# cfpark00/vdm4cdm

Measured on NVIDIA B200. Metric: denoiser voxel-steps/s at 128^3 (reverse ancestral sampling), higher is better.
Workload: dtype bf16

## Files before the change

__graft_entry__.py:

```python
from __future__ import annotations

import os
import subprocess
import sys

ROOT = os.path.dirname(os.path.abspath(__file__))
if ROOT not in sys.path:
    sys.path.insert(0, ROOT)


def build() -> None:
    subprocess.run(["make", "-C", os.path.join(ROOT, "vdm4cdm_b200", "csrc"), "-j", "8"], check=True)
    os.makedirs(os.path.join(ROOT, "tools", "bin"), exist_ok=True)
    subprocess.run(["nvcc", "-gencode", "arch=compute_100a,code=sm_100a", "-O3", "-std=c++17", "-lineinfo", "-o",
                    os.path.join(ROOT, "tools", "bin", "probe_umma"), os.path.join(ROOT, "tools", "probe_umma.cu")],
                   check=True)
    import vdm4cdm_b200
    from vdm4cdm_b200 import _C
    lib = _C.lib()
    missing = [n for n in _C.declared_symbols() if not hasattr(lib, n)]
    if missing:
        raise RuntimeError(f"libvdm4cdm_b200.so does not export {missing}")
    import oracle


def smoke() -> None:
    import numpy as np
    import torch

    from oracle import power_ref
    from oracle.unet_ref import CUNet as RefNet
    from oracle.vdm_ref import VDM as RefVDM
    from vdm4cdm_b200 import _C, utils
    from vdm4cdm_b200.networks import CUNet
    from vdm4cdm_b200.vdm_model import VDM

    _C.check(_C.lib().vdm_device_supported(0), "vdm_device_supported")
    torch.manual_seed(0)
    shape, chs, b = (1, 16, 16, 16), (16, 32), 2
    kw = dict(shape=shape, chs=chs, s_conditioning_channels=1, v_conditioning_dims=[6], t_conditioning=True)
    ref = RefNet(**kw).eval()
    net = CUNet(**kw)
    net.load_state_dict(ref.state_dict())
    net = net.cuda().eval()
    g = torch.Generator().manual_seed(1)
    x = torch.randn((b,) + shape, generator=g)
    cond = 0.7 * x + 0.3 * torch.randn((b,) + shape, generator=g)
    t = torch.rand(b, generator=g)
    v = [torch.rand(b, 6, generator=g)]
    with torch.no_grad():
        want = ref(x, t=t, s_conditioning=cond, v_conditionings=v)
        got = net(x.cuda(), t=t.cuda(), s_conditioning=cond.cuda(), v_conditionings=[v[0].cuda()]).cpu()
    err = ((got - want).norm() / want.norm()).item()
    assert err < 1e-2, f"denoiser output differs from the oracle: relative L2 {err}"

    noises = [torch.randn((b,) + shape, generator=g) for _ in range(4)]
    vdm, ref_vdm = VDM(net).cuda().eval(), RefVDM(ref).eval()
    xs = vdm.sample(b, 3, "cuda:0", noise_fn=lambda d, s: noises[d].cuda(), s_conditioning=cond.cuda(),
                    v_conditionings=[v[0].cuda()]).cpu()
    with torch.no_grad():
        xr = ref_vdm.sample(b, 3, "cpu", noise_fn=lambda d, s: noises[d], s_conditioning=cond, v_conditionings=v)
    err_s = ((xs - xr).norm() / xr.norm()).item()
    assert err_s < 5e-2, f"3-step sample differs from the oracle: relative L2 {err_s}"

    from oracle.vdm_ref import LightVDM as RefLight
    from vdm4cdm_b200.vdm_model import LightVDM
    ref_l, mod_l = RefLight(ref).train(), LightVDM(net).cuda().train()
    for m in (ref, net):
        for blk in m.modules():
            if isinstance(blk, torch.nn.Dropout):
                blk.p = 0.0
    net.dropout_prob = 0.0
    for _, blk in net._blocks():
        blk.dropout_prob = 0.0
    times = torch.tensor([0.3, 0.8])
    loss_r, _ = ref_l.get_loss({"x": x, "conditioning": cond, "conditioning_values": v}, noise=noises[0], noise0=noises[1], times=times)
    loss_r.backward()
    loss_c, _ = mod_l.get_loss({"x": x.cuda(), "conditioning": cond.cuda(), "conditioning_values": [v[0].cuda()]},
                               noise=noises[0].cuda(), noise0=noises[1].cuda(), times=times.cuda())
    loss_c.backward()
    num = den = 0.0
    refp = dict(ref_l.named_parameters())
    for n_, p_ in mod_l.named_parameters():
        if p_.grad is not None and refp[n_].grad is not None:
            num += (p_.grad.cpu() - refp[n_].grad).double().pow(2).sum().item()
            den += refp[n_].grad.double().pow(2).sum().item()
    err_g = (num / den) ** 0.5
    assert abs(loss_c.item() - loss_r.item()) < 1e-2 * abs(loss_r.item()), (loss_c.item(), loss_r.item())
    assert err_g < 3e-2, f"training gradients differ from oracle autograd: relative L2 {err_g}"

    f1 = np.random.default_rng(2).standard_normal((2, 1, 32, 32, 32), dtype=np.float32)
    f2 = (0.7 * f1 + 0.3 * np.random.default_rng(3).standard_normal(f1.shape, dtype=np.float32)).astype(np.float32)
    k, p, n = utils.pk(torch.from_numpy(f1).cuda())
    ko, po, no = power_ref.pk(f1)
    assert np.array_equal(n.cpu().numpy(), no) and np.allclose(p.cpu().numpy(), po, rtol=1e-5)
    _, cc = utils.get_ccs(torch.from_numpy(f1).cuda(), torch.from_numpy(f2).cuda())
    assert np.allclose(cc.cpu().numpy(), power_ref.get_ccs(f1, f2)[1], atol=2e-5)
    torch.cuda.synchronize()
    print(f"smoke ok: denoiser rel-L2 {err:.2e}, 3-step sample rel-L2 {err_s:.2e}, VDM loss {loss_c.item():.4f} vs {loss_r.item():.4f}, "
          f"gradient rel-L2 {err_g:.2e}, P(k)/r(k) match")


if __name__ == "__main__":
    build()
    import torch
    if torch.cuda.is_available():
        smoke()
```

vdm4cdm_b200/csrc/conv3d.cu:

```cuda
#include "common.cuh"
#include "ptx.cuh"
#include "tma_host.cuh"

#ifdef VDM_BRINGUP
#define VDM_DBG(p, f) (((p).debug_flags & (f)) != 0)
#else
#define VDM_DBG(p, f) (false)
#endif

namespace vdm {

constexpr int kConvThreads = 512;
constexpr int kEpiThreads = 256;
constexpr int kEpiFirst = 128;
constexpr int kXfThreads = 128;
constexpr int kXfFirst = 384;
constexpr int kRegsWg0 = 64, kRegsEpi = 176, kRegsXf = 88;
constexpr int kXfGroup = 2;
constexpr int kResSlotBytes = 2 * 16 * kEpiThreads;
constexpr int kMaxBStages = 16;
constexpr int kMaxAStages = 4;
constexpr int kTileH = 16, kTileW = 8;

struct ConvKernelParams {
  int B, D, H, W;
  int c_out;
  int n_cta, n_split;
  int n_pad;
  int n_taps, pad;
  uint16_t tap16[VDM_MAX_TAPS];
  int8_t tap_kd[VDM_MAX_TAPS];
  int8_t tap_khw[VDM_MAX_TAPS];
  int8_t tap_of[3][9];
  int fold_streamed;
  int MT, KC, k_chunks;
  int Hd, Hh, Wh;
  int tiles_w, tiles_h, tiles_d, n_tiles;
  int fast_div_ok;
  float inv_n_split, inv_tiles_w, inv_tiles_h, inv_tiles_d;
  int a_stage_bytes, b_stage_bytes, nsb, taps_per_stage;
  int nsa;
  int b_resident;
  int plane_bytes;
  int tmem_cols;
  int x_planes, x_plane0, c_in8;
  int x_shift;
  int skip_chunks;
  int x2_planes, x2_plane0;
  int skip_w_bytes;
  const __nv_bfloat16* w2;
  const __nv_bfloat16* w;
  void* y;
  int y_planes, y_plane0, out_fp32;
  const float* chan_add;
  const int32_t* step_ptr;
  long long chan_add_step_stride;
  const __nv_bfloat16* residual;
  int r_planes, r_plane0;
  int r_up;
  int r_d2s_planes;
  int res_depth;
  int res_ring_off;
  double* stats;
  int stats_channels, stats_c0;
  const float* in_norm;
  int c_in;
  int xf_coef_off;
  int m_units, m_nseg, m_seglen;
  int debug_flags;
};

struct ConvShared {
  uint64_t a_full[kMaxAStages], a_empty[kMaxAStages];
  uint64_t a_ready[kMaxAStages];
  uint64_t b_full[kMaxBStages], b_empty[kMaxBStages];
  uint64_t tmem_full[2], tmem_empty[2];
  uint32_t tmem_base;
  alignas(16) float cadd[2][256];
};

__device__ __forceinline__ void warp_column_sums16(float (&v)[16]) {
  const unsigned full = 0xffffffffu;
  const int lane = threadIdx.x & 31;
#pragma unroll
  for (int i = 0; i < 8; ++i) {
    const bool hi = lane & 16;
    const float send = hi ? v[i] : v[i + 8];
    const float keep = hi ? v[i + 8] : v[i];
    v[i] = keep + __shfl_xor_sync(full, send, 16);
  }
#pragma unroll
  for (int i = 0; i < 4; ++i) {
    const bool hi = lane & 8;
    const float send = hi ? v[i] : v[i + 4];
    const float keep = hi ? v[i + 4] : v[i];
    v[i] = keep + __shfl_xor_sync(full, send, 8);
  }
#pragma unroll
  for (int i = 0; i < 2; ++i) {
    const bool hi = lane & 4;
    const float send = hi ? v[i] : v[i + 2];
    const float keep = hi ? v[i + 2] : v[i];
    v[i] = keep + __shfl_xor_sync(full, send, 4);
  }
  {
    const bool hi = lane & 2;
    const float send = hi ? v[0] : v[1];
    const float keep = hi ? v[1] : v[0];
    v[0] = keep + __shfl_xor_sync(full, send, 2);
  }
  v[0] += __shfl_xor_sync(full, v[0], 1);
}

struct TileCoord {
  int b, d0, h0, w0, ns;
};
__device__ __forceinline__ int fast_div(int x, int d, float inv) {
  (void)d;
  return __float2int_rz(((float)x + 0.5f) * inv);
}
__device__ __forceinline__ TileCoord decode_tile(const ConvKernelParams& p, int tile) {
  TileCoord t;
  int q;
  if (p.fast_div_ok) {
    q = fast_div(tile, p.n_split, p.inv_n_split); t.ns = tile - q * p.n_split; tile = q;
    q = fast_div(tile, p.tiles_w, p.inv_tiles_w); t.w0 = (tile - q * p.tiles_w) * kTileW; tile = q;
    q = fast_div(tile, p.tiles_h, p.inv_tiles_h); t.h0 = (tile - q * p.tiles_h) * kTileH; tile = q;
    q = fast_div(tile, p.tiles_d, p.inv_tiles_d); t.d0 = (tile - q * p.tiles_d) * p.MT;
    t.b = q;
  } else {
    t.ns = tile % p.n_split; tile /= p.n_split;
    t.w0 = (tile % p.tiles_w) * kTileW; tile /= p.tiles_w;
    t.h0 = (tile % p.tiles_h) * kTileH; tile /= p.tiles_h;
    t.d0 = (tile % p.tiles_d) * p.MT;
    t.b = tile / p.tiles_d;
  }
  return t;
}

struct Ring {
  uint32_t s, ph, n;
  __device__ __forceinline__ explicit Ring(uint32_t n_) : s(0u), ph(0u), n(n_) {}
  __device__ __forceinline__ void next() {
    if (++s == n) {
      s = 0u;
      ph ^= 1u;
    }
  }
};
__device__ __forceinline__ uint32_t hold_u32(uint32_t v) {
  asm volatile("mov.u32 %0, %0;" : "+r"(v));
  return v;
}

__device__ __forceinline__ uint64_t make_planar_desc(uint32_t smem_addr, uint32_t lbo, uint32_t sbo) {
  uint64_t d = 0;
  d |= (uint64_t)((smem_addr & 0x3FFFFu) >> 4);
  d |= (uint64_t)((lbo >> 4) & 0x3FFFu) << 16;
  d |= (uint64_t)((sbo >> 4) & 0x3FFFu) << 32;
  d |= (uint64_t)1 << 46;
  return d;
}

template <int MT, int KJ, int NF, bool FIRST>
__device__ __forceinline__ void issue_fold_tile(uint32_t a_lo0, uint32_t b_base16, uint64_t a_hi, uint64_t b_hi,
                                                uint32_t d_tmem0) {
  constexpr int Hh = kTileH + 2, Wh = kTileW + 2, Hd = MT + 2;
  constexpr uint32_t plane16 = (uint32_t)(Hd * Hh * Wh);
  constexpr uint32_t kstep_a16 = 2u * plane16;
  const uint32_t a_hi32 = (uint32_t)(a_hi >> 32), b_hi32 = (uint32_t)(b_hi >> 32);
#pragma unroll 1
  for (int i = 0; i < MT + 2; ++i) {
    const int kd_lo = (i - MT + 1) > 0 ? (i - MT + 1) : 0;
    const int kd_hi = i < 2 ? i : 2;
    const int s_lo = i - kd_hi;
    const int nblk = kd_hi - kd_lo + 1;
    const bool starts = FIRST && i < MT;
    const uint32_t a_i = a_lo0 + (uint32_t)(i * Hh * Wh) + (uint32_t)a_hi;
    const uint32_t b_i = b_base16 + (uint32_t)((2 - kd_hi) * NF) + (uint32_t)b_hi;
    const uint32_t d_i = d_tmem0 + (uint32_t)(s_lo * NF);
    const uint32_t idesc_i = ptx::make_idesc_bf16(128, (uint32_t)(nblk * NF));
#pragma unroll
    for (int khw = 0; khw < 9; ++khw) {
#pragma unroll
      for (int j = 0; j < KJ; ++j) {
        const uint32_t a_off = (uint32_t)((khw / 3) * Wh + khw % 3) + (uint32_t)j * kstep_a16;
        const uint32_t b_off = (uint32_t)((khw * 2 * KJ + 2 * j) * 3 * NF);
        if (khw == 0 && j == 0) {
          if (starts) {
            if (nblk > 1)
              ptx::umma_bf16_off(d_i, 0u, a_i, a_off, a_hi32, b_i, b_off, b_hi32,
                                 ptx::make_idesc_bf16(128, (uint32_t)((nblk - 1) * NF)), 1u);
            ptx::umma_bf16_off(d_tmem0, (uint32_t)(i * NF), a_i, a_off, a_hi32, b_i, b_off + (uint32_t)((nblk - 1) * NF), b_hi32,
                               ptx::make_idesc_bf16(128, (uint32_t)NF), 0u);
          } else {
            ptx::umma_bf16_off(d_i, 0u, a_i, a_off, a_hi32, b_i, b_off, b_hi32, idesc_i, 1u);
          }
        } else {
          ptx::umma_bf16_off(d_i, 0u, a_i, a_off, a_hi32, b_i, b_off, b_hi32, idesc_i, 1u);
        }
      }
    }
  }
}

template <int MT, int KJ, int NF>
__device__ __forceinline__ void issue_skip_chunk(uint32_t a_lo0, uint32_t b_lo16, uint32_t d_tmem0) {
  constexpr uint32_t slice16 = (uint32_t)(kTileH * kTileW);
  constexpr uint32_t plane16 = (uint32_t)MT * slice16;
  constexpr uint32_t kstep_a16 = 2u * plane16;
  const uint64_t a_hi = make_planar_desc(0, plane16 * 16u, (uint32_t)kTileW * 16u);
  const uint64_t b_hi = make_planar_desc(0, (uint32_t)NF * 16u, 128u);
  const uint32_t a_hi32 = (uint32_t)(a_hi >> 32), b_hi32 = (uint32_t)(b_hi >> 32);
  const uint32_t idesc = ptx::make_idesc_bf16(128, (uint32_t)NF);
  const uint32_t b_i = b_lo16 + (uint32_t)b_hi;
#pragma unroll
  for (int i = 0; i < MT; ++i) {
    const uint32_t a_i = a_lo0 + (uint32_t)i * slice16 + (uint32_t)a_hi;
#pragma unroll
    for (int j = 0; j < KJ; ++j)
      ptx::umma_bf16_off(d_tmem0, (uint32_t)(i * NF), a_i, (uint32_t)j * kstep_a16, a_hi32, b_i, (uint32_t)(2 * j * NF),
                         b_hi32, idesc, 1u);
  }
}

template <int MT, int KJ, int NF>
__device__ __forceinline__ void issue_fold_stage(uint32_t a_lo, uint32_t b_lo, uint32_t a_hi32, uint32_t b_hi32,
                                                 uint32_t d_tmem0, bool first) {
  constexpr int Hh = kTileH + 2, Wh = kTileW + 2, Hd = MT + 2;
  constexpr uint32_t plane16 = (uint32_t)(Hd * Hh * Wh);
  constexpr uint32_t kstep_a16 = 2u * plane16;
#pragma unroll
  for (int i = 0; i < MT + 2; ++i) {
    const int kd_lo = (i - MT + 1) > 0 ? (i - MT + 1) : 0;
    const int kd_hi = i < 2 ? i : 2;
    const int s_lo = i - kd_hi;
    const int nblk = kd_hi - kd_lo + 1;
#pragma unroll
    for (int j = 0; j < KJ; ++j) {
      const uint32_t a_off = (uint32_t)(i * Hh * Wh) + (uint32_t)j * kstep_a16;
      const uint32_t b_off = (uint32_t)((2 * j * 3 + (2 - kd_hi)) * NF);
      if (j == 0 && i < MT && first) {
        if (nblk > 1)
          ptx::umma_bf16_off(d_tmem0, (uint32_t)(s_lo * NF), a_lo, a_off, a_hi32, b_lo, b_off, b_hi32,
                             ptx::make_idesc_bf16(128, (uint32_t)((nblk - 1) * NF)), 1u);
        ptx::umma_bf16_off(d_tmem0, (uint32_t)(i * NF), a_lo, a_off, a_hi32, b_lo, b_off + (uint32_t)((nblk - 1) * NF), b_hi32,
                           ptx::make_idesc_bf16(128, (uint32_t)NF), 0u);
      } else {
        ptx::umma_bf16_off(d_tmem0, (uint32_t)(s_lo * NF), a_lo, a_off, a_hi32, b_lo, b_off, b_hi32,
                           ptx::make_idesc_bf16(128, (uint32_t)(nblk * NF)), 1u);
      }
    }
  }
}

template <int HH, int WH>
__device__ __forceinline__ bool halo_voxel_oob(int v, int dlo, int hlo, int wlo, int D, int H, int W) {
  const int dz = v / (HH * WH);
  const int rem = v - dz * (HH * WH);
  const int hy = rem / WH;
  const int wx = rem - hy * WH;
  return (unsigned)(dlo + dz) >= (unsigned)D || (unsigned)(hlo + hy) >= (unsigned)H || (unsigned)(wlo + wx) >= (unsigned)W;
}

__device__ __forceinline__ uint4 gn_silu8(const uint4 x, const float (&ca)[8], const float (&cb)[8]) {
  bf16x8 in;
  in.u = x;
  float f[8];
  unpack8(in, f);
#pragma unroll
  for (int j = 0; j < 8; ++j) {
    const float h = fmaf(f[j], ca[j], cb[j]);
    float t;
    asm("tanh.approx.f32 %0, %1;" : "=f"(t) : "f"(h));
    f[j] = fmaf(h, t, h);
  }
  return pack8(f).u;
}

template <int MT, int KJ>
__device__ __forceinline__ void transform_tiles(const ConvKernelParams& p, ConvShared* sh, uint8_t* a_smem, float* coef) {
  constexpr int planes = 2 * KJ;
  constexpr int nparts = planes >= 4 ? 1 : 4 / planes;
  static_assert((MT + 2) * (kTileH + 2) * (kTileW + 2) <= 64 * 32, "zmask: one bit per 16-byte unit of a thread");
  constexpr int pl_step = planes >= 4 ? 4 : planes;
  const int xt = threadIdx.x - kXfFirst, tw = xt >> 5, lane = xt & 31;
  const int pl0 = planes >= 4 ? tw : tw % planes;
  const int part = planes >= 4 ? 0 : tw / planes;
  const int vh = p.Hd * p.Hh * p.Wh;
  const int total_chunks = p.k_chunks + p.skip_chunks;
  int cur_b = -1;
  Ring ra((uint32_t)p.nsa);
  for (int tile = blockIdx.x; tile < p.n_tiles; tile += gridDim.x) {
    const TileCoord t = decode_tile(p, tile);
    if (t.b != cur_b) {
      asm volatile("bar.sync 3, 128;" ::: "memory");
      const float4* src = reinterpret_cast<const float4*>(p.in_norm + (long long)t.b * p.c_in * 2);
      for (int i = xt; i < p.c_in / 2; i += kXfThreads) reinterpret_cast<float4*>(coef)[i] = __ldg(src + i);
      asm volatile("bar.sync 3, 128;" ::: "memory");
      cur_b = t.b;
    }
    const int dlo = t.d0 - p.pad + p.x_shift, hlo = t.h0 - p.pad + p.x_shift, wlo = t.w0 - p.pad + p.x_shift;
    unsigned long long zmask = 0ull;
    if (dlo < 0 || dlo + p.Hd > p.D || hlo < 0 || hlo + p.Hh > p.H || wlo < 0 || wlo + p.Wh > p.W) {
      int k = 0;
      for (int idx = part * 32 + lane; idx < vh; idx += 32 * nparts, ++k) {
        const bool oob = p.pad ? halo_voxel_oob<kTileH + 2, kTileW + 2>(idx, dlo, hlo, wlo, p.D, p.H, p.W)
                               : halo_voxel_oob<kTileH, kTileW>(idx, dlo, hlo, wlo, p.D, p.H, p.W);
        if (oob) zmask |= 1ull << k;
      }
    }
    for (int kc = 0; kc < total_chunks; ++kc, ra.next()) {
      const int s = (int)ra.s;
      ptx::mbar_wait(&sh->a_full[s], ra.ph);
      if (kc < p.k_chunks && !VDM_DBG(p, 64)) {
        uint8_t* stage = a_smem + (size_t)s * p.a_stage_bytes;
#pragma unroll 1
        for (int pl = pl0; pl < planes; pl += pl_step) {
          float ca[8], cb[8];
          {
            const float4* cs = reinterpret_cast<const float4*>(coef + (size_t)((kc * planes + pl) * 8) * 2);
#pragma unroll
            for (int j4 = 0; j4 < 4; ++j4) {
              const float4 c4 = cs[j4];
              ca[2 * j4] = c4.x; cb[2 * j4] = c4.y; ca[2 * j4 + 1] = c4.z; cb[2 * j4 + 1] = c4.w;
            }
          }
          uint4* base = reinterpret_cast<uint4*>(stage + (size_t)pl * p.plane_bytes);
          constexpr int G = kXfGroup;
          const int step = 32 * nparts;
          int v = part * 32 + lane;
          uint4 cur[G], nxt[G];
#pragma unroll
          for (int g2 = 0; g2 < G; ++g2) {
            const int idx = v + g2 * step;
            cur[g2] = idx < vh ? base[idx] : make_uint4(0u, 0u, 0u, 0u);
          }
          int k = 0;
#pragma unroll 1
          for (; v < vh; v += G * step, k += G) {
            const int vn = v + G * step;
#pragma unroll
            for (int g2 = 0; g2 < G; ++g2) {
              const int idx = vn + g2 * step;
              nxt[g2] = idx < vh ? base[idx] : make_uint4(0u, 0u, 0u, 0u);
            }
            const unsigned zk = (unsigned)(zmask >> k);
#pragma unroll
            for (int g2 = 0; g2 < G; ++g2) {
              const int idx = v + g2 * step;
              uint4 y = VDM_DBG(p, 128) ? cur[g2] : gn_silu8(cur[g2], ca, cb);
              if ((zk >> g2) & 1u) y = make_uint4(0u, 0u, 0u, 0u);
              if (idx < vh && !VDM_DBG(p, 256)) base[idx] = y;
            }
#pragma unroll
            for (int g2 = 0; g2 < G; ++g2) cur[g2] = nxt[g2];
          }
        }
      }
      ptx::fence_proxy_async();
      ptx::mbar_arrive(&sh->a_ready[s]);
    }
  }
}

constexpr int kEpiRes = 1, kEpiStats = 2, kEpiFp32 = 4;
constexpr int kEpiF32Planar = 8;

template <int MT, int MODE>
__device__ __forceinline__ void epilogue_tiles(const ConvKernelParams& p, ConvShared* sh, uint8_t* smem, float* stat_part,
                                               double* stat_acc, const uint32_t tmem_base) {
  constexpr bool RES = (MODE & kEpiRes) != 0, STATS = (MODE & kEpiStats) != 0, FP32 = (MODE & kEpiFp32) != 0;
  constexpr bool F32P = (MODE & kEpiF32Planar) != 0;
  constexpr int kUnitPlanes = F32P ? 4 : 2;
  constexpr int kPlaneShift = F32P ? 2 : 3;
  const int warp = threadIdx.x >> 5, lane = threadIdx.x & 31;
  const int q = warp & 3;
  const int ew = warp - (kEpiFirst >> 5);
  const int half = ew >> 2;
  const int et = threadIdx.x - kEpiFirst;
  const int r = q * 32 + lane;
  const int lh = r >> 3, lw = r & 7;
  const int n_cta = p.n_cta;
  const int n_chunks = n_cta >> 4;
  const bool split_ch = n_chunks >= 2;
  const int ch0 = split_ch ? half : 0, ch_step = split_ch ? 2 : 1;
  const int s0 = split_ch ? 0 : half, s_step = split_ch ? 1 : 2;
  const long long HW = (long long)p.H * p.W, V = (long long)p.D * HW;
  float* cadd_tab = &sh->cadd[0][0];
  const bool cadd_table = p.B * p.n_pad <= 512;
  const long long cadd_step = (p.chan_add && p.step_ptr) ? (long long)(*p.step_ptr) : 0ll;
  const float* cadd_g = p.chan_add ? p.chan_add + cadd_step * p.chan_add_step_stride : nullptr;
  if (cadd_table) {
    for (int i = et; i < p.B * p.n_pad; i += kEpiThreads) {
      const int bb = i / p.n_pad, c = i - bb * p.n_pad;
      cadd_tab[i] = (cadd_g && c < p.c_out) ? __ldg(cadd_g + (long long)bb * p.c_out + c) : 0.f;
    }
    asm volatile("bar.sync 1, 256;" ::: "memory");
  }
  constexpr int kResPrefetchTiles = 3;
  const int r_depth = p.res_depth;
  uint4* r_ring = reinterpret_cast<uint4*>(smem + p.res_ring_off) + et;
  int r_slot = 0;
  const uint4* res_base = reinterpret_cast<const uint4*>(p.residual);
  const int r_sh = p.r_up;
  const int r_H = p.H >> r_sh, r_W = p.W >> r_sh;
  const long long r_HW = (long long)r_H * r_W, r_V = (long long)(p.D >> r_sh) * r_HW;
  int r_tile = blockIdx.x - (int)gridDim.x;
  int ru_s = 0, ru_ch = n_chunks;
  const uint4* r_ptr = nullptr;
  int r_d0 = 0, r_cbase = 0;
  bool r_hw_ok = false;
  auto res_issue = [&](int slot) __attribute__((always_inline)) {
    bool live = true;
    if (ru_ch >= n_chunks) {
      r_tile += (int)gridDim.x;
      if (r_tile < p.n_tiles) {
        const TileCoord tr = decode_tile(p, r_tile);
        const int hr = tr.h0 + lh, wr = tr.w0 + lw;
        r_hw_ok = (hr < p.H) && (wr < p.W);
        r_d0 = tr.d0;
        r_cbase = tr.ns * n_cta;
        r_ptr = res_base + ((long long)tr.b * p.r_planes + p.r_plane0 + (r_cbase >> kPlaneShift) +
                            (((hr & 1) << 1) | (wr & 1)) * p.r_d2s_planes) * r_V +
                (long long)(hr >> r_sh) * r_W + (wr >> r_sh);
        ru_s = s0; ru_ch = ch0;
      } else {
        live = false;
      }
    }
    if (live) {
      const int su = ru_s, chu = ru_ch;
      ru_s += s_step;
      if (ru_s >= MT) { ru_s = s0; ru_ch += ch_step; }
      if (r_hw_ok && r_d0 + su < p.D) {
        const uint4* src = r_ptr + (long long)(chu * kUnitPlanes + (((r_d0 + su) & 1) << 2) * p.r_d2s_planes) * r_V +
                           (long long)((r_d0 + su) >> r_sh) * r_HW;
        const int cu = r_cbase + chu * 16;
        uint4* dst = r_ring + (kUnitPlanes * slot) * kEpiThreads;
        if constexpr (F32P) {
#pragma unroll
          for (int k = 0; k < 4; ++k)
            if (cu + 4 * k < p.c_out) ptx::cp_async16(dst + k * kEpiThreads, src + k * r_V);
        } else {
          if (cu < p.c_out) ptx::cp_async16(dst, src);
          if (cu + 8 < p.c_out) ptx::cp_async16(dst + kEpiThreads, src + r_V);
        }
      }
    }
    ptx::cp_async_commit();
  };
  if (RES) {
    for (int i = 0; i < r_depth; ++i) res_issue(i);
  }
  uint32_t ti = 0;
  for (int tile = blockIdx.x; tile < p.n_tiles; tile += gridDim.x, ++ti) {
    const TileCoord t = decode_tile(p, tile);
    const int h = t.h0 + lh, w = t.w0 + lw;
    const bool hw_ok = (h < p.H) && (w < p.W);
    const int cbase = t.ns * n_cta;
    const uint32_t acc = ti & 1;
    if (RES && p.r_d2s_planes == 0) {
      const int pt = tile + kResPrefetchTiles * (int)gridDim.x;
      if (pt < p.n_tiles) {
        const TileCoord tp = decode_tile(p, pt);
        const int pc0 = tp.ns * n_cta;
        const int n_rows = (n_cta >> kPlaneShift) * MT * 16;
        const uint4* pbase = res_base + ((long long)tp.b * p.r_planes + p.r_plane0 + (pc0 >> kPlaneShift)) * r_V + (tp.w0 >> r_sh);
        for (int idx = et; idx < n_rows; idx += kEpiThreads) {
          const int hh = tp.h0 + (idx & 15);
          const int sp_ = idx >> 4;
          const int pp = sp_ / MT;
          const int dd = tp.d0 + (sp_ - pp * MT);
          if (hh < p.H && dd < p.D && pc0 + (pp << kPlaneShift) < p.c_out && !(r_sh && ((hh | dd) & 1)))
            ptx::prefetch_l2(pbase + (long long)pp * r_V + ((long long)(dd >> r_sh) * r_H + (hh >> r_sh)) * r_W);
        }
      }
    }
    const int buf = ti & 1;
    if (!cadd_table) {
      if (et < n_cta)
        sh->cadd[buf][et] = (cadd_g && cbase + et < p.c_out) ? __ldg(cadd_g + (long long)t.b * p.c_out + cbase + et) : 0.f;
      asm volatile("bar.sync 1, 256;" ::: "memory");
    }
    const float* cadd_row = cadd_tab + (cadd_table ? t.b * p.n_pad + cbase : buf * 256);
    const long long vox0 = ((long long)t.d0 * p.H + h) * p.W + w;
    float* sp = stat_part + (ti & 1) * (16 * n_cta);
    ptx::mbar_wait(&sh->tmem_full[acc], (ti >> 1) & 1);
    ptx::tc_fence_after();
    const uint32_t trow0 = tmem_base + ((uint32_t)(q * 32) << 16) + (uint32_t)(acc * MT * n_cta);
    bool released = false;
    for (int ch = ch0; ch < n_chunks; ch += ch_step) {
      const int c0 = cbase + ch * 16;
      const bool last_chunk = ch + ch_step >= n_chunks;
      const int c_left = p.c_out - c0;
      const int nhf = c_left >= 16 ? 2 : (c_left >= 8 ? 1 : 0);
      float cb[16];
      {
        const float4* cs = reinterpret_cast<const float4*>(cadd_row + ch * 16);
#pragma unroll
        for (int j4 = 0; j4 < 4; ++j4) {
          const float4 cv = cs[j4];
          cb[4 * j4] = cv.x; cb[4 * j4 + 1] = cv.y; cb[4 * j4 + 2] = cv.z; cb[4 * j4 + 3] = cv.w;
        }
      }
      float s1[16], s2[16];
      if (STATS) {
#pragma unroll
        for (int j = 0; j < 16; ++j) s1[j] = s2[j] = 0.f;
      }
      bf16x8* y_ch = reinterpret_cast<bf16x8*>(p.y) + ((long long)t.b * p.y_planes + p.y_plane0 + (c0 >> 3)) * V + vox0;
      float* y32_ch = static_cast<float*>(p.y) + ((long long)t.b * p.c_out + c0) * V + vox0;
      float4* y4_ch = static_cast<float4*>(p.y) + ((long long)t.b * p.y_planes + p.y_plane0 + (c0 >> 2)) * V + vox0;
      auto process = [&](uint32_t (&raw)[16], int s) __attribute__((always_inline)) {
        const bool valid = hw_ok && (t.d0 + s < p.D);
        uint4 rcur0 = make_uint4(0, 0, 0, 0), rcur1 = make_uint4(0, 0, 0, 0);
        uint4 rcur2 = make_uint4(0, 0, 0, 0), rcur3 = make_uint4(0, 0, 0, 0);
        if (RES) {
          ptx::cp_async_wait(r_depth - 1);
          const uint4* slot = r_ring + (kUnitPlanes * r_slot) * kEpiThreads;
          rcur0 = slot[0]; rcur1 = slot[kEpiThreads];
          if (F32P) { rcur2 = slot[2 * kEpiThreads]; rcur3 = slot[3 * kEpiThreads]; }
          res_issue(r_slot);
          r_slot = (r_slot + 1 == r_depth) ? 0 : r_slot + 1;
        }
        float f[16];
#pragma unroll
        for (int j = 0; j < 16; j += 2) {
          f[j] = __uint_as_float(raw[j]); f[j + 1] = __uint_as_float(raw[j + 1]);
          add2(f[j], f[j + 1], cb[j], cb[j + 1]);
        }
        if (FP32) {
          if (valid) {
            float* yp = y32_ch + (long long)s * HW;
#pragma unroll
            for (int j = 0; j < 16; ++j)
              if (j < c_left) yp[(long long)j * V] = f[j];
          }
          return;
        }
        if (nhf == 0 || !valid) return;
        if (F32P) {
          float4* yp = y4_ch + (long long)s * HW;
#pragma unroll
          for (int hf = 0; hf < 2; ++hf) {
            if (hf == 1 && nhf < 2) break;
            float g[8];
#pragma unroll
            for (int j = 0; j < 8; ++j) g[j] = f[hf * 8 + j];
            if (RES) {
              const uint4 ra = hf == 0 ? rcur0 : rcur2, rb = hf == 0 ? rcur1 : rcur3;
              add2(g[0], g[1], __uint_as_float(ra.x), __uint_as_float(ra.y));
              add2(g[2], g[3], __uint_as_float(ra.z), __uint_as_float(ra.w));
              add2(g[4], g[5], __uint_as_float(rb.x), __uint_as_float(rb.y));
              add2(g[6], g[7], __uint_as_float(rb.z), __uint_as_float(rb.w));
            }
            yp[(long long)(2 * hf) * V] = make_float4(g[0], g[1], g[2], g[3]);
            yp[(long long)(2 * hf + 1) * V] = make_float4(g[4], g[5], g[6], g[7]);
            if (STATS) {
#pragma unroll
              for (int j = 0; j < 8; j += 2) {
                add2(s1[hf * 8 + j], s1[hf * 8 + j + 1], g[j], g[j + 1]);
                fma2_sq(s2[hf * 8 + j], s2[hf * 8 + j + 1], g[j], g[j + 1]);
              }
            }
          }
          return;
        }
        bf16x8* yp = y_ch + (long long)s * HW;
#pragma unroll
        for (int hf = 0; hf < 2; ++hf) {
          if (hf == 1 && nhf < 2) break;
          float g[8];
#pragma unroll
          for (int j = 0; j < 8; ++j) g[j] = f[hf * 8 + j];
          if (RES) {
            float rr[8];
            bf16x8 rv;
            rv.u = hf == 0 ? rcur0 : rcur1;
            unpack8(rv, rr);
#pragma unroll
            for (int j = 0; j < 8; j += 2) add2(g[j], g[j + 1], rr[j], rr[j + 1]);
          }
          const bf16x8 packed = pack8(g);
          yp[hf == 0 ? 0 : V] = packed;
          if (STATS) {
            unpack8(packed, g);
#pragma unroll
            for (int j = 0; j < 8; j += 2) {
              add2(s1[hf * 8 + j], s1[hf * 8 + j + 1], g[j], g[j + 1]);
              fma2_sq(s2[hf * 8 + j], s2[hf * 8 + j + 1], g[j], g[j + 1]);
            }
          }
        }
      };
      const uint32_t tcol = trow0 + (uint32_t)(ch * 16);
      uint32_t raw_a[16], raw_b[16];
      int s = s0;
      if (s < MT) ptx::tmem_ld16(tcol + (uint32_t)(s * n_cta), raw_a);
#pragma unroll
      for (int i = 0; i < MT; ++i) {
        if (s >= MT) break;
        const int sn = s + s_step;
        if ((i & 1) == 0) {
          ptx::tmem_ld_wait_dep(raw_a);
          if (sn < MT) ptx::tmem_ld16(tcol + (uint32_t)(sn * n_cta), raw_b);
        } else {
          ptx::tmem_ld_wait_dep(raw_b);
          if (sn < MT) ptx::tmem_ld16(tcol + (uint32_t)(sn * n_cta), raw_a);
        }
        if (last_chunk && sn >= MT) {
          ptx::tc_fence_before();
          ptx::mbar_arrive(&sh->tmem_empty[acc]);
          released = true;
        }
        if ((i & 1) == 0) process(raw_a, s);
        else process(raw_b, s);
        s = sn;
      }
      if (STATS && nhf > 0) {
        warp_column_sums16(s1);
        warp_column_sums16(s2);
        if ((lane & 1) == 0) {
          const int c = ch * 16 + (lane >> 1);
          sp[ew * n_cta + c] = s1[0];
          sp[(8 + ew) * n_cta + c] = s2[0];
        }
      }
    }
    if (!released) {
      ptx::tc_fence_before();
      ptx::mbar_arrive(&sh->tmem_empty[acc]);
    }
    if (STATS) {
      asm volatile("bar.sync 2, 256;" ::: "memory");
      if (et < n_cta) {
        const int next_tile = tile + (int)gridDim.x;
        bool flush = next_tile >= p.n_tiles;
        if (!flush) {
          const TileCoord tn = decode_tile(p, next_tile);
          flush = (tn.b != t.b) || (tn.ns != t.ns);
        }
        const int c = et;
        float t1 = 0.f, t2 = 0.f;
#pragma unroll
        for (int wv = 0; wv < 8; ++wv) {
          t1 += sp[wv * n_cta + c];
          t2 += sp[(8 + wv) * n_cta + c];
          sp[wv * n_cta + c] = 0.f;
          sp[(8 + wv) * n_cta + c] = 0.f;
        }
        const double a1 = stat_acc[c] + (double)t1;
        const double a2 = stat_acc[n_cta + c] + (double)t2;
        if (flush) {
          if (cbase + c < p.c_out) {
            double* dst = p.stats + ((long long)t.b * p.stats_channels + p.stats_c0 + cbase + c) * 2;
            atomicAdd(dst, a1);
            atomicAdd(dst + 1, a2);
          }
          stat_acc[c] = 0.0;
          stat_acc[n_cta + c] = 0.0;
        } else {
          stat_acc[c] = a1;
          stat_acc[n_cta + c] = a2;
        }
      }
    }
  }
}

template <int MT, int KJ, int PAD, int TPS, bool RESIDENT, ptx::MmaKind KIND>
__device__ __forceinline__ void issue_generic_tiles(const ConvKernelParams& p, ConvShared* sh, uint64_t* a_rdy, uint32_t a_base16,
                                                    uint32_t b_base16, uint32_t tmem_u, bool leader) {
  constexpr uint32_t Hh = kTileH + 2 * PAD, Wh = kTileW + 2 * PAD, Hd = MT + 2 * PAD;
  constexpr uint32_t slice16 = Hh * Wh;
  constexpr uint32_t kstep_a16 = 2u * Hd * Hh * Wh;
  const uint32_t n_cta = hold_u32((uint32_t)p.n_cta);
  const uint32_t idesc = ptx::make_idesc_bf16<KIND>(128, n_cta);
  const uint64_t a_hi = make_planar_desc(0, Hd * Hh * Wh * 16u, Wh * 16u);
  const uint64_t b_hi = make_planar_desc(0, n_cta * 16u, 128u);
  const uint32_t a_stage16 = hold_u32((uint32_t)p.a_stage_bytes >> 4), b_stage16 = hold_u32((uint32_t)p.b_stage_bytes >> 4);
  const uint32_t kstep_b16 = 2u * n_cta;
  const uint32_t btap16 = (uint32_t)(2 * KJ) * n_cta;
  constexpr int tps = TPS;
  constexpr bool resident = RESIDENT;
  const int n_taps = (int)hold_u32((uint32_t)p.n_taps);
  const int k_chunks = (int)hold_u32((uint32_t)p.k_chunks);
  Ring ra(hold_u32((uint32_t)p.nsa)), rb(hold_u32((uint32_t)p.nsb));
  uint32_t ti = 0;
  bool first_chunk = true;
  for (int tile = blockIdx.x; tile < p.n_tiles; tile += gridDim.x, ++ti) {
    const uint32_t acc = ti & 1;
    ptx::mbar_wait(&sh->tmem_empty[acc], ((ti >> 1) & 1) ^ 1);
    ptx::tc_fence_after();
    const uint32_t d_tmem0 = tmem_u + acc * (uint32_t)MT * n_cta;
    for (int kc = 0; kc < k_chunks; ++kc, ra.next()) {
      const uint32_t sa = ra.s;
      ptx::mbar_wait(&a_rdy[sa], ra.ph);
      if (resident && first_chunk) ptx::mbar_wait(&sh->b_full[0], 0);
      first_chunk = false;
      ptx::tc_fence_after();
      const uint32_t a_lo0 = a_base16 + sa * a_stage16;
      if (leader) {
        for (int tap0 = 0; tap0 < n_taps; tap0 += tps) {
          uint32_t b_lo0;
          if (resident) {
            b_lo0 = b_base16 + (uint32_t)(kc * n_taps + tap0) * btap16;
          } else {
            ptx::mbar_wait(&sh->b_full[rb.s], rb.ph);
            ptx::tc_fence_after();
            b_lo0 = b_base16 + rb.s * b_stage16;
          }
#pragma unroll
          for (int q = 0; q < tps; ++q) {
            const uint64_t a_tap = a_hi | (uint64_t)(a_lo0 + (uint32_t)p.tap16[tap0 + q]);
            const uint32_t first = (kc | tap0 | q) != 0 ? 1u : 0u;
            uint64_t b_tap[KJ];
#pragma unroll
            for (int j = 0; j < KJ; ++j) b_tap[j] = b_hi | (uint64_t)(b_lo0 + (uint32_t)q * btap16 + (uint32_t)j * kstep_b16);
#pragma unroll
            for (int s = 0; s < MT; ++s) {
#pragma unroll
              for (int j = 0; j < KJ; ++j)
                ptx::umma_bf16_off64<KIND>(d_tmem0, (uint32_t)s * n_cta, a_tap, (uint32_t)s * slice16 + (uint32_t)j * kstep_a16, b_tap[j],
                                           0u, idesc, j == 0 ? first : 1u);
            }
          }
          if (!resident) {
            ptx::umma_commit(&sh->b_empty[rb.s]);
            rb.next();
          }
        }
        ptx::umma_commit(&sh->a_empty[sa]);
        if (kc == k_chunks - 1) ptx::umma_commit(&sh->tmem_full[acc]);
      }
      __syncwarp();
    }
  }
}

template <int MT, int KJ, int NF, bool TF32 = false>
__global__ void __launch_bounds__(kConvThreads, 1)
conv3d_planar_kernel(const __grid_constant__ CUtensorMap tmap_x, const __grid_constant__ CUtensorMap tmap_x2,
                     const __grid_constant__ ConvKernelParams p) {
  static_assert(!TF32 || NF == 0, "the TF32 instances run the generic schedule only");
  constexpr ptx::MmaKind kKind = TF32 ? ptx::MmaKind::kTF32 : ptx::MmaKind::kF16;
  extern __shared__ __align__(1024) uint8_t smem_raw[];
  uint8_t* smem = smem_raw + ((1024u - (ptx::smem_u32(smem_raw) & 1023u)) & 1023u);
  uint8_t* a_smem = smem;
  uint8_t* b_smem = smem + (size_t)p.nsa * p.a_stage_bytes;
  ConvShared* sh = reinterpret_cast<ConvShared*>(b_smem + (size_t)p.nsb * p.b_stage_bytes + p.skip_w_bytes);
  constexpr bool kFold = NF > 0;

  const int warp = threadIdx.x >> 5;
  const int lane = threadIdx.x & 31;

  if (threadIdx.x == 0) {
    ptx::prefetch_tensormap(&tmap_x);
    for (int s = 0; s < kMaxAStages; ++s) {
      ptx::mbar_init(&sh->a_full[s], 1);
      ptx::mbar_init(&sh->a_empty[s], 1);
      ptx::mbar_init(&sh->a_ready[s], kXfThreads);
    }
    for (int s = 0; s < 2; ++s) {
      ptx::mbar_init(&sh->tmem_full[s], 1);
      ptx::mbar_init(&sh->tmem_empty[s], kEpiThreads);
    }
    for (int s = 0; s < p.nsb && s < kMaxBStages; ++s) {
      ptx::mbar_init(&sh->b_full[s], 1);
      ptx::mbar_init(&sh->b_empty[s], 1);
    }
    ptx::fence_barrier_init();
  }
  if (warp == 1) {
    ptx::tmem_alloc(&sh->tmem_base, (uint32_t)p.tmem_cols);
    ptx::tmem_relinquish();
  }
  float* stat_part = reinterpret_cast<float*>(sh + 1);
  double* stat_acc = reinterpret_cast<double*>(stat_part + 2 * 2 * 8 * p.n_cta);
  if (warp >= 4 && warp < 12) {
    for (int i = threadIdx.x - kEpiFirst; i < 2 * p.n_cta; i += kEpiThreads) stat_acc[i] = 0.0;
    for (int i = threadIdx.x - kEpiFirst; i < 2 * 2 * 8 * p.n_cta; i += kEpiThreads) stat_part[i] = 0.f;
  }
  ptx::tc_fence_before();
  __syncthreads();
  ptx::tc_fence_after();
  const uint32_t tmem_base = sh->tmem_base;
  constexpr int planes_per_chunk = KJ * 2;
  uint64_t* const a_rdy = p.in_norm ? sh->a_ready : sh->a_full;
  if (warp < 4) {
  ptx::setmaxnreg_dec<kRegsWg0>();

  if (warp == 0) {
    if (lane == 0) {
      uint32_t it = 0;
      Ring ra((uint32_t)p.nsa);
      for (int tile = blockIdx.x; tile < p.n_tiles; tile += gridDim.x) {
        const TileCoord t = decode_tile(p, tile);
        for (int kc = 0; kc < p.k_chunks + p.skip_chunks; ++kc, ++it, ra.next()) {
          const int s = (int)ra.s;
          ptx::mbar_wait(&sh->a_empty[s], ra.ph ^ 1u);
          if (VDM_DBG(p, 2) && it >= 2) {
            ptx::mbar_arrive(&sh->a_full[s]);
            continue;
          }
          if (kc < p.k_chunks) {
            ptx::mbar_arrive_expect_tx(&sh->a_full[s], (uint32_t)(planes_per_chunk * p.plane_bytes));
            ptx::tma_load_4d(a_smem + (size_t)s * p.a_stage_bytes, &tmap_x, &sh->a_full[s], (t.w0 - p.pad + p.x_shift) * 8,
                             t.h0 - p.pad + p.x_shift, t.d0 - p.pad + p.x_shift,
                             t.b * p.x_planes + p.x_plane0 + kc * planes_per_chunk);
          } else {
            ptx::mbar_arrive_expect_tx(&sh->a_full[s], (uint32_t)(planes_per_chunk * MT * kTileH * kTileW * 16));
            ptx::tma_load_4d(a_smem + (size_t)s * p.a_stage_bytes, &tmap_x2, &sh->a_full[s], t.w0 * 8, t.h0, t.d0,
                             t.b * p.x2_planes + p.x2_plane0 + (kc - p.k_chunks) * planes_per_chunk);
          }
        }
      }
    }
  } else if (warp == 2 || warp == 3) {
    const uint32_t pj = (uint32_t)(warp - 2);
    const bool streamed = kFold ? p.fold_streamed != 0 : p.b_resident == 0;
    if (lane == 0 && blockIdx.x < (unsigned)p.n_tiles && (pj == 0 || streamed)) {
      const uint32_t plane_copy_bytes = (uint32_t)p.n_cta * 16u;
      const int tps = p.taps_per_stage, nsb = p.nsb, n_taps = p.n_taps, k_chunks = p.k_chunks;
      const size_t tap_stride = (size_t)p.c_in8 * p.n_pad * 8, plane_stride = (size_t)p.n_pad * 8;
      if constexpr (kFold) {
       if (p.fold_streamed) {
        Ring rb((uint32_t)nsb);
        uint32_t n_st = 0;
        for (int tile = blockIdx.x; tile < p.n_tiles; tile += gridDim.x)
          for (int kc = 0; kc < k_chunks; ++kc)
            for (int khw = 0; khw < 9; ++khw, rb.next(), ++n_st) {
              if ((n_st & 1u) != pj) continue;
              const int s = (int)rb.s;
              ptx::mbar_wait(&sh->b_empty[s], rb.ph ^ 1u);
              ptx::mbar_arrive_expect_tx(&sh->b_full[s], plane_copy_bytes * planes_per_chunk * 3u);
              uint8_t* dst = b_smem + (size_t)s * p.b_stage_bytes;
#pragma unroll
              for (int kd = 0; kd < 3; ++kd) {
                const __nv_bfloat16* src = p.w + (size_t)p.tap_of[kd][khw] * tap_stride + (size_t)kc * planes_per_chunk * plane_stride;
#pragma unroll
                for (int pl = 0; pl < planes_per_chunk; ++pl)
                  ptx::bulk_load(dst + (size_t)(pl * 3 + (2 - kd)) * plane_copy_bytes, src + (size_t)pl * plane_stride,
                                 plane_copy_bytes, &sh->b_full[s]);
              }
            }
       } else {
        ptx::mbar_arrive_expect_tx(&sh->b_full[0], plane_copy_bytes * planes_per_chunk * (uint32_t)(n_taps * k_chunks) +
                                                       (uint32_t)p.skip_w_bytes);
        for (int kc = 0; kc < k_chunks; ++kc)
          for (int tap = 0; tap < n_taps; ++tap) {
            const int kd = p.tap_kd[tap], khw = p.tap_khw[tap];
#pragma unroll
            for (int pl = 0; pl < planes_per_chunk; ++pl)
              ptx::bulk_load(b_smem + (size_t)(((kc * 9 + khw) * planes_per_chunk + pl) * 3 + (2 - kd)) * plane_copy_bytes,
                             p.w + (size_t)tap * tap_stride + (size_t)(kc * planes_per_chunk + pl) * plane_stride,
                             plane_copy_bytes, &sh->b_full[0]);
          }
        for (int pl = 0; pl < p.skip_chunks * planes_per_chunk; ++pl)
          ptx::bulk_load(b_smem + (size_t)p.b_stage_bytes + (size_t)pl * plane_copy_bytes, p.w2 + (size_t)pl * plane_stride,
                         plane_copy_bytes, &sh->b_full[0]);
       }
      } else if (p.b_resident) {
        const uint32_t total = plane_copy_bytes * planes_per_chunk * (uint32_t)(n_taps * k_chunks);
        ptx::mbar_arrive_expect_tx(&sh->b_full[0], total);
        for (int kc = 0; kc < k_chunks; ++kc)
          for (int tap = 0; tap < n_taps; ++tap) {
            uint8_t* dst = b_smem + (size_t)(kc * n_taps + tap) * planes_per_chunk * plane_copy_bytes;
            const __nv_bfloat16* src = p.w + (size_t)tap * tap_stride + (size_t)kc * planes_per_chunk * p.n_pad * 8;
#pragma unroll
            for (int pl = 0; pl < planes_per_chunk; ++pl)
              ptx::bulk_load(dst + (size_t)pl * plane_copy_bytes, src + (size_t)pl * plane_stride, plane_copy_bytes,
                             &sh->b_full[0]);
          }
      } else {
        Ring rb((uint32_t)nsb);
        const bool whole_rows = p.n_split == 1;
        const uint32_t stage_tx = plane_copy_bytes * (uint32_t)planes_per_chunk * (uint32_t)tps;
        const uint32_t tap_bytes = plane_copy_bytes * (uint32_t)planes_per_chunk;
        const size_t chunk_stride = (size_t)planes_per_chunk * plane_stride;
        const uint32_t b_stage_bytes = (uint32_t)p.b_stage_bytes;
        uint32_t n_st = 0;
        for (int tile = blockIdx.x; tile < p.n_tiles; tile += gridDim.x) {
          const TileCoord t = decode_tile(p, tile);
          const __nv_bfloat16* src_c = p.w + (size_t)t.ns * p.n_cta * 8;
          for (int kc = 0; kc < k_chunks; ++kc, src_c += chunk_stride) {
            const __nv_bfloat16* src = src_c;
            for (int tap0 = 0; tap0 < n_taps; tap0 += tps, rb.next(), ++n_st) {
              if ((n_st & 1u) != pj) {
                src += (size_t)tps * tap_stride;
                continue;
              }
              const uint32_t s = rb.s;
              ptx::mbar_wait(&sh->b_empty[s], rb.ph ^ 1u);
              ptx::mbar_arrive_expect_tx(&sh->b_full[s], stage_tx);
              uint8_t* dst = b_smem + (size_t)s * b_stage_bytes;
              if (whole_rows) {
                for (int q = 0; q < tps; ++q, src += tap_stride, dst += tap_bytes) ptx::bulk_load(dst, src, tap_bytes, &sh->b_full[s]);
              } else {
                for (int q = 0; q < tps; ++q, src += tap_stride)
#pragma unroll
                  for (int pl = 0; pl < planes_per_chunk; ++pl, dst += plane_copy_bytes)
                    ptx::bulk_load(dst, src + (size_t)pl * plane_stride, plane_copy_bytes, &sh->b_full[s]);
              }
            }
          }
        }
      }
    }
  } else if (warp == 1) {
    const uint32_t n_cta = (uint32_t)p.n_cta;
    const uint32_t a_base16 = ptx::smem_u32(a_smem) >> 4, a_stage16 = (uint32_t)p.a_stage_bytes >> 4;
    const uint32_t nsa_u = (uint32_t)p.nsa;
    const uint32_t b_base16 = ptx::smem_u32(b_smem) >> 4, b_stage16 = (uint32_t)p.b_stage_bytes >> 4;
    const uint32_t tmem_u = __shfl_sync(0xffffffffu, tmem_base, 0);
    const bool leader = ptx::elect_one();
    const uint64_t a_hi = make_planar_desc(0, (uint32_t)p.plane_bytes, (uint32_t)p.Wh * 16u);
    if constexpr (kFold) {
      const uint64_t b_hi = make_planar_desc(0, 3u * (uint32_t)NF * 16u, 128u);
      constexpr uint32_t chunk_b16 = 9u * 2u * KJ * 3u * NF;
      const int k_chunks = p.k_chunks;
      uint32_t ti = 0;
      if (p.fold_streamed) {
        const uint32_t a_hi32 = (uint32_t)(a_hi >> 32), b_hi32 = (uint32_t)(b_hi >> 32);
        const uint32_t a_lbo = (uint32_t)a_hi, b_lbo = (uint32_t)b_hi;
        const uint32_t b_stage16 = hold_u32((uint32_t)p.b_stage_bytes >> 4);
        Ring ra(nsa_u), rb((uint32_t)p.nsb);
        for (int tile = blockIdx.x; tile < p.n_tiles; tile += gridDim.x, ++ti) {
          const uint32_t acc = ti & 1;
          ptx::mbar_wait(&sh->tmem_empty[acc], ((ti >> 1) & 1) ^ 1);
          const uint32_t d_tmem0 = tmem_u + acc * (uint32_t)(MT * NF);
          for (int kc = 0; kc < k_chunks; ++kc, ra.next()) {
            const uint32_t sa = ra.s;
            ptx::mbar_wait(&a_rdy[sa], ra.ph);
            ptx::tc_fence_after();
            const uint32_t a_st = a_base16 + sa * a_stage16 + a_lbo;
            if (leader) {
              for (int khw = 0; khw < 9; ++khw, rb.next()) {
                const uint32_t sb = rb.s;
                ptx::mbar_wait(&sh->b_full[sb], rb.ph);
                ptx::tc_fence_after();
                const uint32_t kh = (uint32_t)khw / 3u, kw = (uint32_t)khw - 3u * kh;
                issue_fold_stage<MT, KJ, NF>(a_st + kh * (uint32_t)(kTileW + 2) + kw, b_base16 + sb * b_stage16 + b_lbo, a_hi32,
                                             b_hi32, d_tmem0, kc == 0 && khw == 0);
                ptx::umma_commit(&sh->b_empty[sb]);
              }
              ptx::umma_commit(&sh->a_empty[sa]);
              if (kc == k_chunks - 1) ptx::umma_commit(&sh->tmem_full[acc]);
            }
            __syncwarp();
          }
        }
      } else {
      Ring ra(nsa_u);
      for (int tile = blockIdx.x; tile < p.n_tiles; tile += gridDim.x, ++ti) {
        const uint32_t acc = ti & 1;
        ptx::mbar_wait(&sh->tmem_empty[acc], ((ti >> 1) & 1) ^ 1);
        if (ti == 0) ptx::mbar_wait(&sh->b_full[0], 0);
        const uint32_t d_tmem0 = tmem_u + acc * (uint32_t)(MT * NF);
        const int total_chunks = k_chunks + p.skip_chunks;
        for (int kc = 0; kc < total_chunks; ++kc, ra.next()) {
          const uint32_t sa = ra.s;
          ptx::mbar_wait(&a_rdy[sa], ra.ph);
          ptx::tc_fence_after();
          if (leader) {
            if (kc == 0)
              issue_fold_tile<MT, KJ, NF, true>(a_base16 + sa * a_stage16, b_base16, a_hi, b_hi, d_tmem0);
            else if (kc < k_chunks)
              issue_fold_tile<MT, KJ, NF, false>(a_base16 + sa * a_stage16, b_base16 + (uint32_t)kc * chunk_b16, a_hi, b_hi,
                                                 d_tmem0);
            else
              issue_skip_chunk<MT, KJ, NF>(a_base16 + sa * a_stage16,
                                           b_base16 + ((uint32_t)p.b_stage_bytes >> 4) + (uint32_t)(kc - k_chunks) * (2u * KJ * NF),
                                           d_tmem0);
            ptx::umma_commit(&sh->a_empty[sa]);
            if (kc == total_chunks - 1) ptx::umma_commit(&sh->tmem_full[acc]);
          }
          __syncwarp();
        }
      }
      }
    } else {
      const bool res = p.b_resident != 0;
      if (!p.pad) {
        if (res) issue_generic_tiles<MT, KJ, 0, 1, true, kKind>(p, sh, a_rdy, a_base16, b_base16, tmem_u, leader);
        else issue_generic_tiles<MT, KJ, 0, 1, false, kKind>(p, sh, a_rdy, a_base16, b_base16, tmem_u, leader);
      } else if (p.taps_per_stage == 3) {
        if (res) issue_generic_tiles<MT, KJ, 1, 3, true, kKind>(p, sh, a_rdy, a_base16, b_base16, tmem_u, leader);
        else issue_generic_tiles<MT, KJ, 1, 3, false, kKind>(p, sh, a_rdy, a_base16, b_base16, tmem_u, leader);
      } else {
        if (res) issue_generic_tiles<MT, KJ, 1, 1, true, kKind>(p, sh, a_rdy, a_base16, b_base16, tmem_u, leader);
        else issue_generic_tiles<MT, KJ, 1, 1, false, kKind>(p, sh, a_rdy, a_base16, b_base16, tmem_u, leader);
      }
    }
  }
  } else if (warp >= 12) {
    ptx::setmaxnreg_dec<kRegsXf>();
    if constexpr (!TF32)
      if (p.in_norm) transform_tiles<MT, KJ>(p, sh, a_smem, reinterpret_cast<float*>(smem + p.xf_coef_off));
  } else {
    ptx::setmaxnreg_inc<kRegsEpi>();
    constexpr int P = TF32 ? kEpiF32Planar : 0;
    if (p.out_fp32) epilogue_tiles<MT, kEpiFp32>(p, sh, smem, stat_part, stat_acc, tmem_base);
    else if (p.residual && p.stats) epilogue_tiles<MT, P | kEpiRes | kEpiStats>(p, sh, smem, stat_part, stat_acc, tmem_base);
    else if (p.residual) epilogue_tiles<MT, P | kEpiRes>(p, sh, smem, stat_part, stat_acc, tmem_base);
    else if (p.stats) epilogue_tiles<MT, P | kEpiStats>(p, sh, smem, stat_part, stat_acc, tmem_base);
    else epilogue_tiles<MT, P>(p, sh, smem, stat_part, stat_acc, tmem_base);
  }

  ptx::tc_fence_before();
  __syncthreads();
  if (warp == 1) {
    ptx::tc_fence_after();
    ptx::tmem_dealloc(tmem_base, (uint32_t)p.tmem_cols);
  }
}

#include "conv3d_march.cuh"

struct ConvOverrides {
  int debug_flags;
  int force_mt, force_kc, force_nsplit;
  int no_resident;
  int no_fold;
  int no_march;
};
#ifdef VDM_BRINGUP
static ConvOverrides g_overrides = {};
#else
constexpr ConvOverrides g_overrides = {};
#endif

enum class ConvSchedule {
  kTile,
  kFoldResident,
  kFoldStreamed,
  kMarch,
};

struct ConvPlan {
  ConvSchedule schedule;
  int pad;
  int mt, kc, n_split, n_cta;
  int n_tiles, grid;
  int nsa, nsb, taps_per_stage;
  int a_stage_bytes, b_stage_bytes, b_resident;
  int res_depth, res_ring_off;
  int xf_coef_off;
  size_t smem_bytes;
  int m_units, m_nseg, m_seglen;
  int debug_flags;
};

static int tap_cell(const VdmConvDesc& d, int t) {
  return (d.tap_offset[t][0] + 1) * 9 + (d.tap_offset[t][1] + 1) * 3 + d.tap_offset[t][2] + 1;
}

static int plan_conv(const VdmConvDesc& d, bool has_residual, bool has_skip, bool has_xf, int skip_c_in, int sms, bool tf32,
                     ConvPlan& pl) {
  const ConvOverrides& ov = g_overrides;
  pl = ConvPlan{};
  pl.debug_flags = ov.debug_flags;
  int pad = 0;
  for (int t = 0; t < d.n_taps; ++t)
    if (d.tap_offset[t][0] != 0 || d.tap_offset[t][1] != 0 || d.tap_offset[t][2] != 0) pad = 1;
  if (has_xf && d.circular) {
    set_error("vdm_conv3d: the fused input transform is not available with circular padding");
    return VDM_E_UNSUPPORTED;
  }
  if (has_skip && (skip_c_in > 64 || d.out_fp32)) {
    set_error("vdm_conv3d: the fused skip conv supports bf16 layers with skip_c_in <= 64 only (got %d)", skip_c_in);
    return VDM_E_UNSUPPORTED;
  }
  const int xf_bytes = has_xf ? ((d.c_in * 8 + 15) & ~15) : 0;
  const int res_slot = tf32 ? 2 * kResSlotBytes : kResSlotBytes;
  const int skip_w_bytes = has_skip ? skip_c_in * d.c_out_pad * 2 : 0;

  bool fold = !tf32 && d.n_taps == 27 && pad == 1 && (d.c_out_pad == 16 || d.c_out_pad == 32 || d.c_out_pad == 64) && d.depth >= 3 &&
              ov.no_fold == 0 && ov.force_mt == 0 && ov.force_nsplit == 0;
  const bool streamed = d.c_out_pad == 64;
  int fold_mt = 0, fold_kc = 0;
  if (fold && streamed) {
    fold = d.c_in % 32 == 0 && d.depth >= 4;
    fold_mt = 4; fold_kc = 32;
  } else if (fold) {
    const int budget = 227 * 1024 - 1024 - (int)sizeof(ConvShared) - (2 * 2 * 8 * d.c_out_pad * 4 + 2 * d.c_out_pad * 8) - 256 -
                       (has_residual ? 2 * res_slot : 0) - xf_bytes;
    const int w_bytes = 27 * d.c_in * d.c_out_pad * 2 + skip_w_bytes;
    for (int m = 4; m >= 2 && !fold_mt; --m)
      for (int c = 32; c >= 16 && !fold_mt; c -= 16) {
        if (d.c_in % c != 0 || (has_skip && skip_c_in % c != 0)) continue;
        const int a_stage = (((c / 8) * (m + 2) * (kTileH + 2) * (kTileW + 2) * 16) + 127) & ~127;
        if (2 * a_stage + w_bytes <= budget) { fold_mt = m; fold_kc = c; }
      }
    fold = fold_mt != 0;
  }
  if (fold) {
    unsigned seen = 0;
    for (int t = 0; t < 27; ++t) seen |= 1u << tap_cell(d, t);
    fold = seen == (1u << 27) - 1u;
  }
  pl.schedule = !fold ? ConvSchedule::kTile : streamed ? ConvSchedule::kFoldStreamed
              : d.c_in == fold_kc && ov.no_march == 0 ? ConvSchedule::kMarch : ConvSchedule::kFoldResident;
  const bool resident_fold = pl.schedule == ConvSchedule::kFoldResident || pl.schedule == ConvSchedule::kMarch;

  const int tiles_w = ceil_div(d.width, kTileW), tiles_h = ceil_div(d.height, kTileH);
  int n_split = 1, mt = fold_mt;
  if (!fold) {
    double best = -1.0;
    for (int ns = 1; ns <= 8; ns *= 2) {
      if (d.c_out_pad % (ns * 16) != 0) break;
      const int ncta = d.c_out_pad / ns;
      if (ns > 1 && ncta < 32) break;
      int mt_max = 256 / ncta;
      if (mt_max > 4) mt_max = 4;
      if (mt_max > d.depth) mt_max = d.depth;
      for (int m = 1; m <= mt_max; ++m) {
        const long long tiles = (long long)tiles_w * tiles_h * ceil_div(d.depth, m) * d.batch * ns;
        const long long waves = (tiles + sms - 1) / sms;
        const double active = (double)(tiles < sms ? tiles : sms);
        const double fetch_cyc = 32.0 + ncta / 4.0;
        const double mma_cyc = (double)d.n_taps * (d.c_in / 16) * m * (ncta / 2.0 > fetch_cyc ? ncta / 2.0 : fetch_cyc);
        const double bytes = (double)(m + 2 * pad) * (kTileH + 2 * pad) * (kTileW + 2 * pad) * d.c_in * 2.0 +
                             (double)d.n_taps * d.c_in * ncta * 2.0;
        double bw = 5500.0 / active;
        if (bw > 64.0) bw = 64.0;
        const double cyc = (mma_cyc > bytes / bw ? mma_cyc : bytes / bw) + 2000.0;
        const double total = (double)waves * cyc;
        if (best < 0.0 || total < best * 0.999) {
          best = total;
          n_split = ns;
          mt = m;
        }
      }
    }
  }
  if (ov.force_nsplit > 0) n_split = ov.force_nsplit;
  VDM_CHECK_ARG(d.c_out_pad % (n_split * 16) == 0, "vdm_conv3d: n_split=%d does not divide c_out_pad=%d", n_split,
                d.c_out_pad);
  const int n_cta = d.c_out_pad / n_split;
  if (ov.force_mt > 0) mt = ov.force_mt;
  VDM_CHECK_ARG(mt >= 1 && 2 * mt * n_cta <= 512, "vdm_conv3d: MT=%d does not fit TMEM with N=%d", mt, n_cta);
  const long long n_tiles = (long long)tiles_w * tiles_h * ceil_div(d.depth, mt) * d.batch * n_split;
  VDM_CHECK_ARG(n_tiles < (1ll << 31), "vdm_conv3d: too many tiles");
  if (has_skip && !resident_fold) {
    set_error("vdm_conv3d: the fused skip conv needs the kd-folded schedule with resident weights "
              "(3x3x3, c_out_pad 16 or 32, weights + skip weights fit shared memory); c_in=%d c_out=%d", d.c_in, d.c_out);
    return VDM_E_UNSUPPORTED;
  }
  pl.pad = pad; pl.mt = mt; pl.n_split = n_split; pl.n_cta = n_cta; pl.n_tiles = (int)n_tiles;
  pl.taps_per_stage = (d.n_taps % 3 == 0) ? 3 : 1;

  if (pl.schedule == ConvSchedule::kMarch) {
    const long long cols = (long long)d.batch * tiles_h * tiles_w;
    int nseg_best = 1;
    double best = -1.0;
    for (int nseg = 1; nseg <= ceil_div(d.depth, 4); ++nseg) {
      const int seglen = ceil_div(d.depth, nseg);
      if (ceil_div(d.depth, seglen) != nseg) continue;
      const long long rounds = (cols * nseg + sms - 1) / sms;
      const double cost = (double)rounds * (seglen + 3);
      if (best < 0.0 || cost < best * 0.999) { best = cost; nseg_best = nseg; }
    }
    const long long units = cols * nseg_best;
    VDM_CHECK_ARG(units < (1ll << 31), "vdm_conv3d: too many units");
    pl.kc = fold_kc;
    pl.m_nseg = nseg_best;
    pl.m_seglen = ceil_div(d.depth, nseg_best);
    pl.m_units = (int)units;
    const int stage_bytes = (fold_kc / 8) * (kTileH + 2) * (kTileW + 2) * 16;
    int off = kMarchStages * stage_bytes + 27 * (fold_kc / 8) * n_cta * 16 + skip_w_bytes + (int)sizeof(MarchShared) +
              2 * kMEpiWarps * n_cta * 4 + 2 * n_cta * 8 + kMarchCaddMax * 4;
    off = (off + 15) & ~15;
    if (has_residual) {
      pl.res_ring_off = off;
      pl.res_depth = kMarchResDepth;
      off += kMarchResDepth * (n_cta / 8) * kMEpiThreads * 16;
    }
    pl.smem_bytes = (size_t)off + 1024;
    VDM_CHECK_ARG(pl.smem_bytes <= 227 * 1024, "vdm_conv3d: marching layer does not fit shared memory");
    pl.grid = pl.m_units < sms ? pl.m_units : sms;
    return VDM_OK;
  }

  const int plane_bytes = (mt + 2 * pad) * (kTileH + 2 * pad) * (kTileW + 2 * pad) * 16;
  const int stat_part_bytes = 2 * 2 * 8 * n_cta * 4 + 2 * n_cta * 8;
  const int smem_total = 227 * 1024 - 1024  - (int)sizeof(ConvShared) - stat_part_bytes - 256 - xf_bytes;
  const int smem_budget = smem_total - (has_residual ? (resident_fold ? 2 : 4) * res_slot : 0);
  if (fold) {
    pl.kc = fold_kc;
    pl.a_stage_bytes = ((fold_kc / 8) * plane_bytes + 127) & ~127;
  }
  if (pl.schedule == ConvSchedule::kFoldStreamed) {
    pl.b_stage_bytes = 3 * fold_kc * n_cta * 2;
    pl.nsb = (smem_budget - 2 * pl.a_stage_bytes) / pl.b_stage_bytes;
    if (pl.nsb > kMaxBStages) pl.nsb = kMaxBStages;
    VDM_CHECK_ARG(pl.nsb >= 2, "vdm_conv3d: folded streamed layer does not fit shared memory");
  } else if (pl.schedule == ConvSchedule::kFoldResident) {
    pl.b_stage_bytes = d.n_taps * d.c_in * n_cta * 2;
    pl.nsb = 1;
    pl.b_resident = 1;
    VDM_CHECK_ARG(2 * pl.a_stage_bytes + pl.b_stage_bytes + skip_w_bytes <= smem_budget,
                  "vdm_conv3d: folded layer does not fit shared memory");
  } else {
    for (int c : {64, 32, 16}) {
      if ((ov.force_kc > 0 && c != ov.force_kc) || d.c_in % c != 0) continue;
      const int a_stage = ((c / 8) * plane_bytes + 127) & ~127;
      const int b_stage = pl.taps_per_stage * c * n_cta * 2;
      const int room = smem_budget - 2 * a_stage;
      if (room < 2 * b_stage) continue;
      const long long all_b = (long long)d.n_taps * d.c_in * n_cta * 2;
      pl.kc = c;
      pl.a_stage_bytes = a_stage;
      pl.b_stage_bytes = b_stage;
      pl.b_resident = (n_split == 1 && all_b <= room && ov.no_resident == 0) ? 1 : 0;
      pl.nsb = pl.b_resident ? (int)((all_b + b_stage - 1) / b_stage) : (room / b_stage > kMaxBStages ? kMaxBStages : room / b_stage);
      break;
    }
    VDM_CHECK_ARG(pl.kc > 0, "vdm_conv3d: no channel-chunk size fits shared memory (c_in=%d, N=%d, MT=%d)", d.c_in, n_cta, mt);
  }
  VDM_CHECK_ARG(plane_bytes <= 0x3FFF * 16, "vdm_conv3d: halo plane too large for the descriptor stride field");

  const int fixed = pl.nsb * pl.b_stage_bytes + skip_w_bytes + (has_residual ? 4 * res_slot : 0);
  pl.nsa = 2;
  while (pl.nsa < kMaxAStages && (pl.nsa + 1) * pl.a_stage_bytes + fixed <= smem_total) ++pl.nsa;
  const int used = pl.nsa * pl.a_stage_bytes + pl.nsb * pl.b_stage_bytes + skip_w_bytes;
  if (has_residual) {
    const int depth = (smem_total - used) / res_slot;
    pl.res_depth = depth > 4 ? 4 : depth;
    VDM_CHECK_ARG(pl.res_depth >= 1, "vdm_conv3d: no shared memory left for the residual ring");
    pl.res_ring_off = (used + (int)sizeof(ConvShared) + stat_part_bytes + 15) & ~15;
  }
  pl.xf_coef_off = (used + (int)sizeof(ConvShared) + stat_part_bytes + 16 + pl.res_depth * res_slot + 15) & ~15;
  pl.smem_bytes = (size_t)pl.xf_coef_off + xf_bytes + 1024;
  pl.grid = pl.n_tiles < sms ? pl.n_tiles : sms;
  return VDM_OK;
}

static int launch_conv(const ConvPlan& pl, const CUtensorMap& tmx, const CUtensorMap& tmx2, const ConvKernelParams& p,
                       bool tf32, cudaStream_t stream) {
  if (pl.schedule == ConvSchedule::kMarch) {
    const bool sk = p.skip_chunks > 0, xf = p.in_norm != nullptr;
#define VDM_MARCH(KJv, NFv, SKv, XFv)                                                                          \
    if (pl.kc == 16 * KJv && pl.n_cta == NFv && sk == SKv && xf == XFv)                                        \
      return launch_kernel<conv3d_march_kernel<KJv, NFv, SKv, XFv>>(pl.grid, kConvThreads, pl.smem_bytes, stream, tmx, tmx2, p);
#define VDM_MARCH4(SKv, XFv) VDM_MARCH(1, 16, SKv, XFv) VDM_MARCH(1, 32, SKv, XFv) VDM_MARCH(2, 16, SKv, XFv) VDM_MARCH(2, 32, SKv, XFv)
    VDM_MARCH4(false, false) VDM_MARCH4(true, false) VDM_MARCH4(false, true) VDM_MARCH4(true, true)
#undef VDM_MARCH4
#undef VDM_MARCH
    set_error("vdm_conv3d: no marching kernel instance for KC=%d N=%d", pl.kc, pl.n_cta);
    return VDM_E_UNSUPPORTED;
  }
  const int nf = pl.schedule == ConvSchedule::kTile ? 0 : pl.n_cta;
  if (tf32) {
#define VDM_TILE_TF32(MTv, KJv)                                                                                \
    if (pl.mt == MTv && pl.kc == 16 * KJv && nf == 0)                                                          \
      return launch_kernel<conv3d_planar_kernel<MTv, KJv, 0, true>>(pl.grid, kConvThreads, pl.smem_bytes, stream, tmx, tmx2, p);
    VDM_TILE_TF32(1, 1) VDM_TILE_TF32(1, 2) VDM_TILE_TF32(1, 4)
    VDM_TILE_TF32(2, 1) VDM_TILE_TF32(2, 2) VDM_TILE_TF32(2, 4)
    VDM_TILE_TF32(3, 1) VDM_TILE_TF32(3, 2) VDM_TILE_TF32(3, 4)
    VDM_TILE_TF32(4, 1) VDM_TILE_TF32(4, 2) VDM_TILE_TF32(4, 4)
#undef VDM_TILE_TF32
    set_error("vdm_conv3d_tf32: no kernel instance for MT=%d KC=%d", pl.mt, pl.kc / 2);
    return VDM_E_UNSUPPORTED;
  }
#define VDM_TILE(MTv, KJv, NFv)                                                                                \
  if (pl.mt == MTv && pl.kc == 16 * KJv && nf == NFv)                                                          \
    return launch_kernel<conv3d_planar_kernel<MTv, KJv, NFv>>(pl.grid, kConvThreads, pl.smem_bytes, stream, tmx, tmx2, p);
  VDM_TILE(1, 1, 0) VDM_TILE(1, 2, 0) VDM_TILE(1, 4, 0)
  VDM_TILE(2, 1, 0) VDM_TILE(2, 2, 0) VDM_TILE(2, 4, 0)
  VDM_TILE(3, 1, 0) VDM_TILE(3, 2, 0) VDM_TILE(3, 4, 0)
  VDM_TILE(4, 1, 0) VDM_TILE(4, 2, 0) VDM_TILE(4, 4, 0)
  VDM_TILE(4, 1, 16) VDM_TILE(4, 1, 32) VDM_TILE(4, 2, 16) VDM_TILE(4, 2, 32) VDM_TILE(4, 2, 64)
  VDM_TILE(3, 1, 16) VDM_TILE(3, 1, 32) VDM_TILE(3, 2, 16) VDM_TILE(3, 2, 32)
  VDM_TILE(2, 1, 16) VDM_TILE(2, 1, 32) VDM_TILE(2, 2, 16) VDM_TILE(2, 2, 32)
#undef VDM_TILE
  set_error("vdm_conv3d: no kernel instance for MT=%d KC=%d", pl.mt, pl.kc);
  return VDM_E_UNSUPPORTED;
}

}

using namespace vdm;

#ifdef VDM_BRINGUP
extern "C" int vdm_debug_set(int key, int value) {
  switch (key) {
    case 0: return VDM_OK;
    case 1: g_overrides.force_mt = value; return VDM_OK;
    case 2: g_overrides.force_kc = value; return VDM_OK;
    case 3: g_overrides.force_nsplit = value; return VDM_OK;
    case 4: g_overrides.no_resident = value; return VDM_OK;
    case 5: g_overrides.debug_flags = value; return VDM_OK;
    case 6: g_overrides.no_fold = value; return VDM_OK;
    case 7: g_overrides.no_march = value; return VDM_OK;
    default: set_error("vdm_debug_set: unknown key %d", key); return VDM_E_BADARG;
  }
}
#endif

static int conv3d_run(const VdmConvDesc& d, const void* x, const void* w, void* y, const VdmConvEpilogue* epi, bool tf32,
                      cudaStream_t stream) {
  VDM_CHECK_ARG(d.batch >= 1 && d.depth >= 1 && d.height >= 1 && d.width >= 1, "vdm_conv3d: bad grid");
  VDM_CHECK_ARG(d.c_in >= 16 && d.c_in % 16 == 0, "vdm_conv3d: c_in=%d must be a multiple of 16", d.c_in);
  VDM_CHECK_ARG(d.c_out_pad >= 16 && d.c_out_pad % 16 == 0 && d.c_out_pad <= 256,
                "vdm_conv3d: c_out_pad=%d must be a multiple of 16 in [16,256]", d.c_out_pad);
  VDM_CHECK_ARG(d.c_out >= 1 && d.c_out <= d.c_out_pad, "vdm_conv3d: c_out=%d vs c_out_pad=%d", d.c_out, d.c_out_pad);
  VDM_CHECK_ARG(d.out_fp32 || d.c_out % 8 == 0, "vdm_conv3d: bf16 planar output needs c_out %% 8 == 0 (got %d)", d.c_out);
  VDM_CHECK_ARG(d.n_taps >= 1 && d.n_taps <= VDM_MAX_TAPS, "vdm_conv3d: n_taps=%d", d.n_taps);
  const int halo = d.circular ? 1 : 0;
  const int x_planes = d.x_planes > 0 ? d.x_planes : d.c_in / 8;
  const int y_planes = d.y_planes > 0 ? d.y_planes : (d.c_out + 7) / 8;
  VDM_CHECK_ARG(d.x_plane0 >= 0 && d.x_plane0 + d.c_in / 8 <= x_planes, "vdm_conv3d: x plane window out of range");
  VDM_CHECK_ARG(d.out_fp32 || (d.y_plane0 >= 0 && d.y_plane0 + d.c_out / 8 <= y_planes),
                "vdm_conv3d: y plane window out of range");
  VDM_CHECK_ARG((reinterpret_cast<uintptr_t>(x) & 15) == 0 && (reinterpret_cast<uintptr_t>(w) & 15) == 0 &&
                    (reinterpret_cast<uintptr_t>(y) & 15) == 0,
                "vdm_conv3d: pointers must be 16-byte aligned");
  VDM_CHECK_ARG((long long)d.batch * x_planes < (1ll << 31), "vdm_conv3d: too many planes");
  for (int t = 0; t < d.n_taps; ++t)
    for (int k = 0; k < 3; ++k)
      VDM_CHECK_ARG(d.tap_offset[t][k] >= -1 && d.tap_offset[t][k] <= 1, "vdm_conv3d: tap offset out of range");
  const bool has_residual = epi && epi->residual;
  const bool has_skip = epi && epi->skip_x;
  const bool has_xf = epi && epi->in_norm;
  VDM_CHECK_ARG(!has_skip || (epi->skip_w && epi->skip_c_in >= 16 && epi->skip_c_in % 16 == 0),
                "vdm_conv3d: fused skip conv needs packed weights and skip_c_in a multiple of 16, got %d", epi->skip_c_in);
  if (!encode_fn()) {
    set_error("vdm_conv3d: cuTensorMapEncodeTiled is not available from the driver");
    return VDM_E_DRIVER;
  }

  ConvPlan pl;
  const int rc = plan_conv(d, has_residual, has_skip, has_xf, has_skip ? epi->skip_c_in : 0, num_sms(), tf32, pl);
  if (rc != VDM_OK) return rc;
  const int x2_planes = !has_skip ? 0 : epi->skip_planes > 0 ? epi->skip_planes : epi->skip_c_in / 8;
  VDM_CHECK_ARG(!has_skip || (epi->skip_plane0 >= 0 && epi->skip_plane0 + epi->skip_c_in / 8 <= x2_planes),
                "vdm_conv3d: skip plane window out of range");
  VDM_CHECK_ARG(!(epi && epi->stats && d.out_fp32), "vdm_conv3d: stats are only produced for bf16 outputs");
  VDM_CHECK_ARG(!(has_residual && d.out_fp32), "vdm_conv3d: residual is only supported for bf16 outputs");
  VDM_CHECK_ARG(!(has_residual && epi->residual_upsample) || (d.depth % 2 == 0 && d.height % 2 == 0 && d.width % 2 == 0),
                "vdm_conv3d: an up-sampled residual needs an even grid, got (%d,%d,%d)", d.depth, d.height, d.width);
  const bool march = pl.schedule == ConvSchedule::kMarch;

  ConvKernelParams p;
  memset(&p, 0, sizeof(p));
  p.B = d.batch; p.D = d.depth; p.H = d.height; p.W = d.width;
  p.c_out = d.c_out; p.n_pad = d.c_out_pad; p.n_taps = d.n_taps; p.pad = pl.pad;
  p.n_split = pl.n_split; p.n_cta = pl.n_cta;
  p.MT = pl.mt; p.KC = pl.kc; p.k_chunks = d.c_in / pl.kc;
  p.tiles_w = ceil_div(d.width, kTileW); p.tiles_h = ceil_div(d.height, kTileH); p.tiles_d = ceil_div(d.depth, pl.mt);
  p.n_tiles = pl.n_tiles;
  p.fast_div_ok = pl.n_tiles < (1 << 22) ? 1 : 0;
  p.inv_n_split = 1.0f / (float)pl.n_split; p.inv_tiles_w = 1.0f / (float)p.tiles_w;
  p.inv_tiles_h = 1.0f / (float)p.tiles_h; p.inv_tiles_d = 1.0f / (float)p.tiles_d;
  p.Hd = pl.mt + 2 * pl.pad; p.Hh = kTileH + 2 * pl.pad; p.Wh = kTileW + 2 * pl.pad;
  p.plane_bytes = p.Hd * p.Hh * p.Wh * 16;
  for (int t = 0; t < d.n_taps; ++t)
    p.tap16[t] = (uint16_t)(((d.tap_offset[t][0] + pl.pad) * p.Hh + (d.tap_offset[t][1] + pl.pad)) * p.Wh + d.tap_offset[t][2] + pl.pad);
  if (pl.schedule != ConvSchedule::kTile)
    for (int t = 0; t < 27; ++t) {
      const int c = tap_cell(d, t);
      p.tap_kd[t] = (int8_t)(c / 9);
      p.tap_khw[t] = (int8_t)(c % 9);
      p.tap_of[c / 9][c % 9] = (int8_t)t;
    }
  p.fold_streamed = pl.schedule == ConvSchedule::kFoldStreamed ? 1 : 0;
  p.nsa = pl.nsa; p.nsb = pl.nsb; p.taps_per_stage = pl.taps_per_stage;
  p.a_stage_bytes = pl.a_stage_bytes; p.b_stage_bytes = pl.b_stage_bytes; p.b_resident = pl.b_resident;
  int cols = 32;
  while (cols < 2 * pl.mt * pl.n_cta) cols <<= 1;
  p.tmem_cols = cols;
  p.c_in = d.c_in; p.c_in8 = d.c_in / 8;
  p.x_planes = x_planes; p.x_plane0 = d.x_plane0;
  p.x_shift = halo;
  if (has_skip) {
    p.skip_chunks = epi->skip_c_in / pl.kc;
    p.skip_w_bytes = epi->skip_c_in * d.c_out_pad * 2;
    p.w2 = static_cast<const __nv_bfloat16*>(epi->skip_w);
    p.x2_planes = x2_planes;
    p.x2_plane0 = epi->skip_plane0;
  }
  p.w = static_cast<const __nv_bfloat16*>(w);
  p.y = y; p.y_planes = y_planes; p.y_plane0 = d.y_plane0; p.out_fp32 = d.out_fp32;
  if (epi) {
    p.chan_add = epi->chan_add;
    p.step_ptr = epi->step_ptr;
    p.chan_add_step_stride = epi->chan_add_step_stride;
    p.residual = static_cast<const __nv_bfloat16*>(epi->residual);
    p.r_planes = d.r_planes > 0 ? d.r_planes : d.c_out / 8;
    p.r_plane0 = d.r_plane0;
    p.r_up = (epi->residual && epi->residual_upsample) ? 1 : 0;
    p.r_d2s_planes = (epi->residual && epi->residual_upsample == 2) ? d.c_out / 8 : 0;
    p.stats = epi->stats;
    p.stats_channels = epi->stats_channels > 0 ? epi->stats_channels : d.c_out;
    p.stats_c0 = epi->stats_c0;
    p.in_norm = epi->in_norm;
  }
  p.res_depth = pl.res_depth; p.res_ring_off = pl.res_ring_off; p.xf_coef_off = pl.xf_coef_off;
  p.m_units = pl.m_units; p.m_nseg = pl.m_nseg; p.m_seglen = pl.m_seglen;
  p.debug_flags = pl.debug_flags;

  const uint32_t box_d = march ? 1u : (uint32_t)p.Hd, planes = (uint32_t)(pl.kc / 8);
  CUtensorMap tmx, tmx2;
  int e = encode_planar(&tmx, x, d.width + 2 * halo, d.height + 2 * halo, d.depth + 2 * halo, (uint64_t)d.batch * x_planes,
                        0, {(uint32_t)p.Wh, (uint32_t)p.Hh, box_d, planes}, "vdm_conv3d", march ? "x, marching" : "x");
  if (e != VDM_OK) return e;
  tmx2 = tmx;
  if (has_skip) {
    e = encode_planar(&tmx2, epi->skip_x, d.width, d.height, d.depth, (uint64_t)d.batch * x2_planes, 0,
                      {(uint32_t)kTileW, (uint32_t)kTileH, march ? 1u : (uint32_t)pl.mt, planes}, "vdm_conv3d",
                      march ? "skip_x, marching" : "skip_x");
    if (e != VDM_OK) return e;
  }
  return launch_conv(pl, tmx, tmx2, p, tf32, stream);
}

extern "C" int vdm_conv3d(const VdmConvDesc* desc, const void* x, const void* w, void* y,
                          const VdmConvEpilogue* epi, void* stream) {
  VDM_CHECK_ARG(desc && x && w && y, "vdm_conv3d: NULL pointer argument");
  return conv3d_run(*desc, x, w, y, epi, false, (cudaStream_t)stream);
}

extern "C" int vdm_conv3d_tf32(const VdmConvDesc* desc, const void* x, const void* w, void* y,
                               const VdmConvEpilogue* epi, void* stream) {
  VDM_CHECK_ARG(desc && x && w && y, "vdm_conv3d_tf32: NULL pointer argument");
  const VdmConvDesc& d = *desc;
  VDM_CHECK_ARG(d.c_in >= 8 && d.c_in % 8 == 0 && d.c_in <= 4096, "vdm_conv3d_tf32: c_in=%d must be a multiple of 8", d.c_in);
  if (epi && (epi->in_norm || epi->skip_x || (epi->residual && epi->residual_upsample))) {
    set_error("vdm_conv3d_tf32: the fused input transform, the fused skip conv and the up-sampled residual are bf16-only");
    return VDM_E_UNSUPPORTED;
  }
  VdmConvDesc d2 = d;
  d2.c_in = 2 * d.c_in;
  if (!d.out_fp32) {
    d2.y_planes = d.y_planes > 0 ? d.y_planes : (d.c_out + 3) / 4;
    VDM_CHECK_ARG(d.y_plane0 >= 0 && d.y_plane0 + d.c_out / 4 <= d2.y_planes, "vdm_conv3d_tf32: y plane window out of range");
  }
  d2.r_planes = d.r_planes > 0 ? d.r_planes : d.c_out / 4;
  return conv3d_run(d2, x, w, y, epi, true, (cudaStream_t)stream);
}
```

vdm4cdm_b200/csrc/ptx.cuh:

```cuda
#pragma once

#include <cuda.h>
#include <stdint.h>

namespace vdm {
namespace ptx {

__device__ __forceinline__ uint32_t smem_u32(const void* p) {
  return static_cast<uint32_t>(__cvta_generic_to_shared(p));
}

__device__ __forceinline__ void mbar_init(uint64_t* bar, uint32_t count) {
  asm volatile("mbarrier.init.shared::cta.b64 [%0], %1;" ::"r"(smem_u32(bar)), "r"(count));
}
__device__ __forceinline__ void fence_barrier_init() {
  asm volatile("fence.mbarrier_init.release.cluster;" ::: "memory");
}
__device__ __forceinline__ void fence_proxy_async() {
  asm volatile("fence.proxy.async.shared::cta;" ::: "memory");
}
__device__ __forceinline__ void mbar_arrive_expect_tx(uint64_t* bar, uint32_t bytes) {
  asm volatile("mbarrier.arrive.expect_tx.shared::cta.b64 _, [%0], %1;" ::"r"(smem_u32(bar)), "r"(bytes)
               : "memory");
}
__device__ __forceinline__ void mbar_arrive(uint64_t* bar) {
  asm volatile("mbarrier.arrive.shared::cta.b64 _, [%0];" ::"r"(smem_u32(bar)) : "memory");
}
__device__ __forceinline__ bool mbar_try_wait(uint64_t* bar, uint32_t parity) {
  uint32_t ok;
  asm volatile(
      "{\n\t"
      ".reg .pred p;\n\t"
      "mbarrier.try_wait.parity.shared::cta.b64 p, [%1], %2;\n\t"
      "selp.u32 %0, 1, 0, p;\n\t"
      "}"
      : "=r"(ok)
      : "r"(smem_u32(bar)), "r"(parity)
      : "memory");
  return ok != 0;
}
__device__ __forceinline__ bool mbar_try_wait_hint(uint64_t* bar, uint32_t parity, uint32_t hint_ns) {
  uint32_t ok;
  asm volatile(
      "{\n\t"
      ".reg .pred p;\n\t"
      "mbarrier.try_wait.parity.shared::cta.b64 p, [%1], %2, %3;\n\t"
      "selp.u32 %0, 1, 0, p;\n\t"
      "}"
      : "=r"(ok)
      : "r"(smem_u32(bar)), "r"(parity), "r"(hint_ns)
      : "memory");
  return ok != 0;
}
__device__ __forceinline__ void mbar_wait(uint64_t* bar, uint32_t parity) {
  if (mbar_try_wait(bar, parity)) return;
  uint32_t spins = 0;
  while (!mbar_try_wait_hint(bar, parity, 2000u)) {
    if (++spins > (1u << 21)) {
      printf("vdm4cdm_b200: mbarrier wait timed out (block %d thread %d)\n", (int)blockIdx.x, (int)threadIdx.x);
      __trap();
    }
  }
}

__device__ __forceinline__ bool elect_one() {
  uint32_t pred;
  asm volatile(
      "{\n\t"
      ".reg .pred p;\n\t"
      "elect.sync _|p, 0xffffffff;\n\t"
      "selp.u32 %0, 1, 0, p;\n\t"
      "}"
      : "=r"(pred));
  return pred != 0;
}

template <int N>
__device__ __forceinline__ void setmaxnreg_inc() {
  asm volatile("setmaxnreg.inc.sync.aligned.u32 %0;" ::"n"(N));
}
template <int N>
__device__ __forceinline__ void setmaxnreg_dec() {
  asm volatile("setmaxnreg.dec.sync.aligned.u32 %0;" ::"n"(N));
}

__device__ __forceinline__ void cp_async16(void* smem_dst, const void* gsrc) {
  asm volatile("cp.async.cg.shared.global [%0], [%1], 16;" ::"r"(smem_u32(smem_dst)), "l"(gsrc) : "memory");
}
__device__ __forceinline__ void cp_async_commit() { asm volatile("cp.async.commit_group;" ::: "memory"); }
__device__ __forceinline__ void cp_async_wait(int pending) {
  switch (pending) {
    case 0: asm volatile("cp.async.wait_group 0;" ::: "memory"); break;
    case 1: asm volatile("cp.async.wait_group 1;" ::: "memory"); break;
    case 2: asm volatile("cp.async.wait_group 2;" ::: "memory"); break;
    default: asm volatile("cp.async.wait_group 3;" ::: "memory"); break;
  }
}

__device__ __forceinline__ void prefetch_l2(const void* p) { asm volatile("prefetch.global.L2 [%0];" ::"l"(p)); }

__device__ __forceinline__ void prefetch_tensormap(const CUtensorMap* m) {
  asm volatile("prefetch.tensormap [%0];" ::"l"(reinterpret_cast<uint64_t>(m)) : "memory");
}
__device__ __forceinline__ void tma_load_5d(void* dst, const CUtensorMap* m, uint64_t* bar, int c0, int c1, int c2,
                                            int c3, int c4) {
  asm volatile(
      "cp.async.bulk.tensor.5d.shared::cluster.global.mbarrier::complete_tx::bytes [%0], [%1, {%3, %4, %5, %6, %7}], "
      "[%2];" ::"r"(smem_u32(dst)),
      "l"(reinterpret_cast<uint64_t>(m)), "r"(smem_u32(bar)), "r"(c0), "r"(c1), "r"(c2), "r"(c3), "r"(c4)
      : "memory");
}
__device__ __forceinline__ void tma_load_4d(void* dst, const CUtensorMap* m, uint64_t* bar, int c0, int c1, int c2,
                                            int c3) {
  asm volatile(
      "cp.async.bulk.tensor.4d.shared::cluster.global.mbarrier::complete_tx::bytes [%0], [%1, {%3, %4, %5, %6}], "
      "[%2];" ::"r"(smem_u32(dst)),
      "l"(reinterpret_cast<uint64_t>(m)), "r"(smem_u32(bar)), "r"(c0), "r"(c1), "r"(c2), "r"(c3)
      : "memory");
}
__device__ __forceinline__ void tma_load_3d(void* dst, const CUtensorMap* m, uint64_t* bar, int c0, int c1, int c2) {
  asm volatile(
      "cp.async.bulk.tensor.3d.shared::cluster.global.mbarrier::complete_tx::bytes [%0], [%1, {%3, %4, %5}], [%2];" ::
          "r"(smem_u32(dst)),
      "l"(reinterpret_cast<uint64_t>(m)), "r"(smem_u32(bar)), "r"(c0), "r"(c1), "r"(c2)
      : "memory");
}

__device__ __forceinline__ void bulk_load(void* dst, const void* src, uint32_t bytes, uint64_t* bar) {
  asm volatile("cp.async.bulk.shared::cluster.global.mbarrier::complete_tx::bytes [%0], [%1], %2, [%3];" ::"r"(
                   smem_u32(dst)),
               "l"(reinterpret_cast<uint64_t>(src)), "r"(bytes), "r"(smem_u32(bar))
               : "memory");
}

__device__ __forceinline__ void tmem_alloc(uint32_t* dst_smem, uint32_t ncols) {
  asm volatile("tcgen05.alloc.cta_group::1.sync.aligned.shared::cta.b32 [%0], %1;" ::"r"(smem_u32(dst_smem)),
               "r"(ncols)
               : "memory");
}
__device__ __forceinline__ void tmem_relinquish() {
  asm volatile("tcgen05.relinquish_alloc_permit.cta_group::1.sync.aligned;" ::: "memory");
}
__device__ __forceinline__ void tmem_dealloc(uint32_t taddr, uint32_t ncols) {
  asm volatile("tcgen05.dealloc.cta_group::1.sync.aligned.b32 %0, %1;" ::"r"(taddr), "r"(ncols) : "memory");
}
__device__ __forceinline__ void tc_fence_before() { asm volatile("tcgen05.fence::before_thread_sync;" ::: "memory"); }
__device__ __forceinline__ void tc_fence_after() { asm volatile("tcgen05.fence::after_thread_sync;" ::: "memory"); }

enum class MmaKind { kF16, kTF32 };
#define VDM_UMMA_KIND_ASM(K, BODY) \
  if constexpr (K == MmaKind::kTF32) asm volatile(BODY("tf32")); else asm volatile(BODY("f16"))

#define VDM_UMMA_BODY(KIND)                                                                    \
      "{\n\t"                                                                                  \
      ".reg .pred p;\n\t"                                                                      \
      "setp.ne.b32 p, %4, 0;\n\t"                                                              \
      "tcgen05.mma.cta_group::1.kind::" KIND " [%0], %1, %2, %3, p;\n\t"                       \
      "}" ::"r"(d_tmem),                                                                       \
      "l"(a_desc), "l"(b_desc), "r"(idesc), "r"(accumulate)                                    \
      : "memory"
template <MmaKind K = MmaKind::kF16>
__device__ __forceinline__ void umma_bf16(uint32_t d_tmem, uint64_t a_desc, uint64_t b_desc, uint32_t idesc,
                                          uint32_t accumulate) {
  VDM_UMMA_KIND_ASM(K, VDM_UMMA_BODY);
}
#undef VDM_UMMA_BODY
#define VDM_UMMA_OFF_BODY(KIND)                                                                \
      "{\n\t"                                                                                  \
      ".reg .pred p;\n\t"                                                                      \
      ".reg .b32 alo, blo, dd;\n\t"                                                            \
      ".reg .b64 da, db;\n\t"                                                                  \
      "add.u32 alo, %1, %2;\n\t"                                                               \
      "add.u32 blo, %4, %5;\n\t"                                                               \
      "add.u32 dd, %0, %9;\n\t"                                                                \
      "mov.b64 da, {alo, %3};\n\t"                                                             \
      "mov.b64 db, {blo, %6};\n\t"                                                             \
      "setp.ne.b32 p, %8, 0;\n\t"                                                              \
      "tcgen05.mma.cta_group::1.kind::" KIND " [dd], da, db, %7, p;\n\t"                       \
      "}" ::"r"(d_tmem),                                                                       \
      "r"(a_lo), "r"(a_off), "r"(a_hi32), "r"(b_lo), "r"(b_off), "r"(b_hi32), "r"(idesc), "r"(accumulate), "r"(d_off) \
      : "memory"
template <MmaKind K = MmaKind::kF16>
__device__ __forceinline__ void umma_bf16_off(uint32_t d_tmem, uint32_t d_off, uint32_t a_lo, uint32_t a_off, uint32_t a_hi32,
                                              uint32_t b_lo, uint32_t b_off, uint32_t b_hi32, uint32_t idesc,
                                              uint32_t accumulate) {
  VDM_UMMA_KIND_ASM(K, VDM_UMMA_OFF_BODY);
}
#undef VDM_UMMA_OFF_BODY
#define VDM_UMMA_OFF64_BODY(KIND)                                                              \
      "{\n\t"                                                                                  \
      ".reg .pred p;\n\t"                                                                      \
      ".reg .b32 dd;\n\t"                                                                      \
      ".reg .b64 da, db;\n\t"                                                                  \
      "add.u64 da, %1, %2;\n\t"                                                                \
      "add.u64 db, %3, %4;\n\t"                                                                \
      "add.u32 dd, %0, %7;\n\t"                                                                \
      "setp.ne.b32 p, %6, 0;\n\t"                                                              \
      "tcgen05.mma.cta_group::1.kind::" KIND " [dd], da, db, %5, p;\n\t"                       \
      "}" ::"r"(d_tmem),                                                                       \
      "l"(a_desc), "l"((uint64_t)a_off), "l"(b_desc), "l"((uint64_t)b_off), "r"(idesc), "r"(accumulate), "r"(d_off) \
      : "memory"
template <MmaKind K = MmaKind::kF16>
__device__ __forceinline__ void umma_bf16_off64(uint32_t d_tmem, uint32_t d_off, uint64_t a_desc, uint32_t a_off, uint64_t b_desc,
                                                uint32_t b_off, uint32_t idesc, uint32_t accumulate) {
  VDM_UMMA_KIND_ASM(K, VDM_UMMA_OFF64_BODY);
}
#undef VDM_UMMA_OFF64_BODY
#undef VDM_UMMA_KIND_ASM
__device__ __forceinline__ void umma_commit(uint64_t* bar) {
  asm volatile("tcgen05.commit.cta_group::1.mbarrier::arrive::one.shared::cluster.b64 [%0];" ::"r"(smem_u32(bar))
               : "memory");
}
__device__ __forceinline__ void tmem_ld16(uint32_t taddr, uint32_t (&r)[16]) {
  asm volatile(
      "tcgen05.ld.sync.aligned.32x32b.x16.b32 {%0, %1, %2, %3, %4, %5, %6, %7, %8, %9, %10, %11, %12, %13, %14, %15}, "
      "[%16];"
      : "=r"(r[0]), "=r"(r[1]), "=r"(r[2]), "=r"(r[3]), "=r"(r[4]), "=r"(r[5]), "=r"(r[6]), "=r"(r[7]), "=r"(r[8]),
        "=r"(r[9]), "=r"(r[10]), "=r"(r[11]), "=r"(r[12]), "=r"(r[13]), "=r"(r[14]), "=r"(r[15])
      : "r"(taddr)
      : "memory");
}
__device__ __forceinline__ void tmem_ld8(uint32_t taddr, uint32_t (&r)[8]) {
  asm volatile("tcgen05.ld.sync.aligned.32x32b.x8.b32 {%0, %1, %2, %3, %4, %5, %6, %7}, [%8];"
               : "=r"(r[0]), "=r"(r[1]), "=r"(r[2]), "=r"(r[3]), "=r"(r[4]), "=r"(r[5]), "=r"(r[6]), "=r"(r[7])
               : "r"(taddr)
               : "memory");
}
__device__ __forceinline__ void tmem_ld_wait() { asm volatile("tcgen05.wait::ld.sync.aligned;" ::: "memory"); }
__device__ __forceinline__ void tmem_ld_wait_dep(uint32_t (&r)[16]) {
  asm volatile("tcgen05.wait::ld.sync.aligned;"
               : "+r"(r[0]), "+r"(r[1]), "+r"(r[2]), "+r"(r[3]), "+r"(r[4]), "+r"(r[5]), "+r"(r[6]), "+r"(r[7]), "+r"(r[8]),
                 "+r"(r[9]), "+r"(r[10]), "+r"(r[11]), "+r"(r[12]), "+r"(r[13]), "+r"(r[14]), "+r"(r[15])
               :
               : "memory");
}

__device__ __forceinline__ uint64_t make_kmajor_desc(uint32_t smem_addr, uint32_t row_bytes) {
  const uint64_t layout = row_bytes == 128 ? 2ull : (row_bytes == 64 ? 4ull : 6ull);
  uint64_t d = 0;
  d |= (uint64_t)((smem_addr & 0x3FFFFu) >> 4);
  d |= (uint64_t)1 << 16;
  d |= (uint64_t)((8u * row_bytes) >> 4) << 32;
  d |= (uint64_t)1 << 46;
  d |= layout << 61;
  return d;
}
template <MmaKind K = MmaKind::kF16>
__device__ __host__ __forceinline__ uint32_t make_idesc_bf16(uint32_t m, uint32_t n) {
  constexpr uint32_t ab = K == MmaKind::kTF32 ? 2u : 1u;
  return (1u << 4) | (ab << 7) | (ab << 10) | ((n >> 3) << 17) | ((m >> 4) << 24);
}

}
}
```

vdm4cdm_b200/csrc/tma_host.cuh:

```cuda
#pragma once

#include <cudaTypedefs.h>

#include "common.cuh"

namespace vdm {

inline PFN_cuTensorMapEncodeTiled_v12000 encode_fn() {
  static PFN_cuTensorMapEncodeTiled_v12000 fn = []() -> PFN_cuTensorMapEncodeTiled_v12000 {
    void* ptr = nullptr;
    cudaDriverEntryPointQueryResult q;
    if (cudaGetDriverEntryPoint("cuTensorMapEncodeTiled", &ptr, cudaEnableDefault, &q) != cudaSuccess ||
        q != cudaDriverEntryPointSuccess)
      return nullptr;
    return reinterpret_cast<PFN_cuTensorMapEncodeTiled_v12000>(ptr);
  }();
  return fn;
}

inline int num_sms() {
  static int n = []() {
    int dev = 0, v = 0;
    if (cudaGetDevice(&dev) != cudaSuccess) return kNumSMs;
    if (cudaDeviceGetAttribute(&v, cudaDevAttrMultiProcessorCount, dev) != cudaSuccess || v <= 0) return kNumSMs;
    return v;
  }();
  return n;
}

struct PlanarBox {
  uint32_t w, h, d, planes;
};

inline int encode_planar(CUtensorMap* map, const void* base, uint64_t W, uint64_t H, uint64_t D, uint64_t batch_planes,
                         int pad, PlanarBox box, const char* who, const char* operand) {
  const uint64_t Wp = W + 2 * pad, Hp = H + 2 * pad, Dp = D + 2 * pad;
  cuuint64_t gdim[4] = {W * 8, H, D, batch_planes};
  cuuint64_t gstr[3] = {Wp * 16, Hp * Wp * 16, Dp * Hp * Wp * 16};
  cuuint32_t bdim[4] = {box.w * 8, box.h, box.d, box.planes};
  cuuint32_t estr[4] = {1, 1, 1, 1};
  const CUresult r = encode_fn()(map, CU_TENSOR_MAP_DATA_TYPE_BFLOAT16, 4, const_cast<void*>(base), gdim, gstr, bdim, estr,
                                 CU_TENSOR_MAP_INTERLEAVE_NONE, CU_TENSOR_MAP_SWIZZLE_NONE,
                                 CU_TENSOR_MAP_L2_PROMOTION_L2_256B, CU_TENSOR_MAP_FLOAT_OOB_FILL_NONE);
  if (r != CUDA_SUCCESS) {
    set_error("%s: cuTensorMapEncodeTiled(%s) failed with %d", who, operand, (int)r);
    return VDM_E_DRIVER;
  }
  return VDM_OK;
}

template <auto Kernel, typename... Args>
int launch_kernel(int grid, int threads, size_t smem_bytes, cudaStream_t stream, const Args&... args) {
  static bool configured = false;
  if (!configured) {
    VDM_CHECK_CUDA(cudaFuncSetAttribute(Kernel, cudaFuncAttributeMaxDynamicSharedMemorySize, 227 * 1024));
    configured = true;
  }
  Kernel<<<grid, threads, smem_bytes, stream>>>(args...);
  VDM_CHECK_LAUNCH();
  return VDM_OK;
}

}
```

Measured before the change: 1.571 billion.

## Add CTA-pair cta_group::2 UMMA path for the generic conv schedule

```diff
diff --git a/__graft_entry__.py b/__graft_entry__.py
--- a/__graft_entry__.py
+++ b/__graft_entry__.py
@@ -10,7 +10,7 @@
 
 
 def build() -> None:
-    subprocess.run(["make", "-C", os.path.join(ROOT, "vdm4cdm_b200", "csrc"), "-j", "8"], check=True)
+    subprocess.run(["make", "-C", os.path.join(ROOT, "vdm4cdm_b200", "csrc"), "-j", "8", "all", "bringup"], check=True)
     os.makedirs(os.path.join(ROOT, "tools", "bin"), exist_ok=True)
     subprocess.run(["nvcc", "-gencode", "arch=compute_100a,code=sm_100a", "-O3", "-std=c++17", "-lineinfo", "-o",
                     os.path.join(ROOT, "tools", "bin", "probe_umma"), os.path.join(ROOT, "tools", "probe_umma.cu")],
diff --git a/vdm4cdm_b200/csrc/conv3d.cu b/vdm4cdm_b200/csrc/conv3d.cu
--- a/vdm4cdm_b200/csrc/conv3d.cu
+++ b/vdm4cdm_b200/csrc/conv3d.cu
@@ -153,6 +153,21 @@
   return v;
 }
 
+template <bool PAIR>
+__device__ __forceinline__ int tiles_run(const ConvKernelParams& p) {
+  return PAIR ? (p.n_tiles + 1) & ~1 : p.n_tiles;
+}
+template <bool PAIR>
+__device__ __forceinline__ void umma_commit_cg(uint64_t* bar) {
+  if constexpr (PAIR) ptx::umma_commit_pair(bar, 3);
+  else ptx::umma_commit(bar);
+}
+template <bool PAIR>
+__device__ __forceinline__ void arrive_leader(uint64_t* bar) {
+  if (PAIR && ptx::cluster_ctarank() != 0) ptx::mbar_arrive_remote(ptx::mapa_shared(bar, 0));
+  else ptx::mbar_arrive(bar);
+}
+
 __device__ __forceinline__ uint64_t make_planar_desc(uint32_t smem_addr, uint32_t lbo, uint32_t sbo) {
   uint64_t d = 0;
   d |= (uint64_t)((smem_addr & 0x3FFFFu) >> 4);
@@ -278,7 +293,7 @@
   return pack8(f).u;
 }
 
-template <int MT, int KJ>
+template <int MT, int KJ, bool PAIR>
 __device__ __forceinline__ void transform_tiles(const ConvKernelParams& p, ConvShared* sh, uint8_t* a_smem, float* coef) {
   constexpr int planes = 2 * KJ;
   constexpr int nparts = planes >= 4 ? 1 : 4 / planes;
@@ -291,8 +306,8 @@
   const int total_chunks = p.k_chunks + p.skip_chunks;
   int cur_b = -1;
   Ring ra((uint32_t)p.nsa);
-  for (int tile = blockIdx.x; tile < p.n_tiles; tile += gridDim.x) {
-    const TileCoord t = decode_tile(p, tile);
+  for (int tile = blockIdx.x; tile < tiles_run<PAIR>(p); tile += gridDim.x) {
+    const TileCoord t = decode_tile(p, PAIR && tile >= p.n_tiles ? p.n_tiles - 1 : tile);
     if (t.b != cur_b) {
       asm volatile("bar.sync 3, 128;" ::: "memory");
       const float4* src = reinterpret_cast<const float4*>(p.in_norm + (long long)t.b * p.c_in * 2);
@@ -359,7 +374,7 @@
         }
       }
       ptx::fence_proxy_async();
-      ptx::mbar_arrive(&sh->a_ready[s]);
+      arrive_leader<PAIR>(&sh->a_ready[s]);
     }
   }
 }
@@ -367,7 +382,7 @@
 constexpr int kEpiRes = 1, kEpiStats = 2, kEpiFp32 = 4;
 constexpr int kEpiF32Planar = 8;
 
-template <int MT, int MODE>
+template <int MT, int MODE, bool PAIR>
 __device__ __forceinline__ void epilogue_tiles(const ConvKernelParams& p, ConvShared* sh, uint8_t* smem, float* stat_part,
                                                double* stat_acc, const uint32_t tmem_base) {
   constexpr bool RES = (MODE & kEpiRes) != 0, STATS = (MODE & kEpiStats) != 0, FP32 = (MODE & kEpiFp32) != 0;
@@ -454,10 +469,11 @@
     for (int i = 0; i < r_depth; ++i) res_issue(i);
   }
   uint32_t ti = 0;
-  for (int tile = blockIdx.x; tile < p.n_tiles; tile += gridDim.x, ++ti) {
-    const TileCoord t = decode_tile(p, tile);
+  for (int tile = blockIdx.x; tile < tiles_run<PAIR>(p); tile += gridDim.x, ++ti) {
+    const bool ghost = PAIR && tile >= p.n_tiles;
+    const TileCoord t = decode_tile(p, ghost ? p.n_tiles - 1 : tile);
     const int h = t.h0 + lh, w = t.w0 + lw;
-    const bool hw_ok = (h < p.H) && (w < p.W);
+    const bool hw_ok = !ghost && (h < p.H) && (w < p.W);
     const int cbase = t.ns * n_cta;
     const uint32_t acc = ti & 1;
     if (RES && p.r_d2s_planes == 0) {
@@ -611,7 +627,7 @@
         }
         if (last_chunk && sn >= MT) {
           ptx::tc_fence_before();
-          ptx::mbar_arrive(&sh->tmem_empty[acc]);
+          arrive_leader<PAIR>(&sh->tmem_empty[acc]);
           released = true;
         }
         if ((i & 1) == 0) process(raw_a, s);
@@ -630,9 +646,9 @@
     }
     if (!released) {
       ptx::tc_fence_before();
-      ptx::mbar_arrive(&sh->tmem_empty[acc]);
-    }
-    if (STATS) {
+      arrive_leader<PAIR>(&sh->tmem_empty[acc]);
+    }
+    if (STATS && !ghost) {
       asm volatile("bar.sync 2, 256;" ::: "memory");
       if (et < n_cta) {
         const int next_tile = tile + (int)gridDim.x;
@@ -669,19 +685,21 @@
   }
 }
 
-template <int MT, int KJ, int PAD, int TPS, bool RESIDENT, ptx::MmaKind KIND>
+template <int MT, int KJ, int PAD, int TPS, bool RESIDENT, ptx::MmaKind KIND, bool PAIR>
 __device__ __forceinline__ void issue_generic_tiles(const ConvKernelParams& p, ConvShared* sh, uint64_t* a_rdy, uint32_t a_base16,
                                                     uint32_t b_base16, uint32_t tmem_u, bool leader) {
   constexpr uint32_t Hh = kTileH + 2 * PAD, Wh = kTileW + 2 * PAD, Hd = MT + 2 * PAD;
   constexpr uint32_t slice16 = Hh * Wh;
   constexpr uint32_t kstep_a16 = 2u * Hd * Hh * Wh;
+  constexpr int CG = PAIR ? 2 : 1;
   const uint32_t n_cta = hold_u32((uint32_t)p.n_cta);
-  const uint32_t idesc = ptx::make_idesc_bf16<KIND>(128, n_cta);
+  const uint32_t n_b = PAIR ? n_cta / 2u : n_cta;
+  const uint32_t idesc = ptx::make_idesc_bf16<KIND>(PAIR ? 256 : 128, n_cta);
   const uint64_t a_hi = make_planar_desc(0, Hd * Hh * Wh * 16u, Wh * 16u);
-  const uint64_t b_hi = make_planar_desc(0, n_cta * 16u, 128u);
+  const uint64_t b_hi = make_planar_desc(0, n_b * 16u, 128u);
   const uint32_t a_stage16 = hold_u32((uint32_t)p.a_stage_bytes >> 4), b_stage16 = hold_u32((uint32_t)p.b_stage_bytes >> 4);
-  const uint32_t kstep_b16 = 2u * n_cta;
-  const uint32_t btap16 = (uint32_t)(2 * KJ) * n_cta;
+  const uint32_t kstep_b16 = 2u * n_b;
+  const uint32_t btap16 = (uint32_t)(2 * KJ) * n_b;
   constexpr int tps = TPS;
   constexpr bool resident = RESIDENT;
   const int n_taps = (int)hold_u32((uint32_t)p.n_taps);
@@ -691,12 +709,12 @@
   bool first_chunk = true;
   for (int tile = blockIdx.x; tile < p.n_tiles; tile += gridDim.x, ++ti) {
     const uint32_t acc = ti & 1;
-    ptx::mbar_wait(&sh->tmem_empty[acc], ((ti >> 1) & 1) ^ 1);
+    ptx::mbar_wait<PAIR>(&sh->tmem_empty[acc], ((ti >> 1) & 1) ^ 1);
     ptx::tc_fence_after();
     const uint32_t d_tmem0 = tmem_u + acc * (uint32_t)MT * n_cta;
     for (int kc = 0; kc < k_chunks; ++kc, ra.next()) {
       const uint32_t sa = ra.s;
-      ptx::mbar_wait(&a_rdy[sa], ra.ph);
+      ptx::mbar_wait<PAIR>(&a_rdy[sa], ra.ph);
       if (resident && first_chunk) ptx::mbar_wait(&sh->b_full[0], 0);
       first_chunk = false;
       ptx::tc_fence_after();
@@ -722,28 +740,30 @@
             for (int s = 0; s < MT; ++s) {
 #pragma unroll
               for (int j = 0; j < KJ; ++j)
-                ptx::umma_bf16_off64<KIND>(d_tmem0, (uint32_t)s * n_cta, a_tap, (uint32_t)s * slice16 + (uint32_t)j * kstep_a16, b_tap[j],
+                ptx::umma_bf16_off64<KIND, CG>(d_tmem0, (uint32_t)s * n_cta, a_tap, (uint32_t)s * slice16 + (uint32_t)j * kstep_a16, b_tap[j],
                                            0u, idesc, j == 0 ? first : 1u);
             }
           }
           if (!resident) {
-            ptx::umma_commit(&sh->b_empty[rb.s]);
+            umma_commit_cg<PAIR>(&sh->b_empty[rb.s]);
             rb.next();
           }
         }
-        ptx::umma_commit(&sh->a_empty[sa]);
-        if (kc == k_chunks - 1) ptx::umma_commit(&sh->tmem_full[acc]);
+        umma_commit_cg<PAIR>(&sh->a_empty[sa]);
+        if (kc == k_chunks - 1) umma_commit_cg<PAIR>(&sh->tmem_full[acc]);
       }
       __syncwarp();
     }
   }
 }
 
-template <int MT, int KJ, int NF, bool TF32 = false>
+template <int MT, int KJ, int NF, bool TF32 = false, bool PAIR = false>
 __global__ void __launch_bounds__(kConvThreads, 1)
 conv3d_planar_kernel(const __grid_constant__ CUtensorMap tmap_x, const __grid_constant__ CUtensorMap tmap_x2,
                      const __grid_constant__ ConvKernelParams p) {
   static_assert(!TF32 || NF == 0, "the TF32 instances run the generic schedule only");
+  static_assert(!PAIR || (NF == 0 && !TF32), "CTA pairs run the bf16 generic schedule only");
+  constexpr int CG = PAIR ? 2 : 1;
   constexpr ptx::MmaKind kKind = TF32 ? ptx::MmaKind::kTF32 : ptx::MmaKind::kF16;
   extern __shared__ __align__(1024) uint8_t smem_raw[];
   uint8_t* smem = smem_raw + ((1024u - (ptx::smem_u32(smem_raw) & 1023u)) & 1023u);
@@ -760,11 +780,11 @@
     for (int s = 0; s < kMaxAStages; ++s) {
       ptx::mbar_init(&sh->a_full[s], 1);
       ptx::mbar_init(&sh->a_empty[s], 1);
-      ptx::mbar_init(&sh->a_ready[s], kXfThreads);
+      ptx::mbar_init(&sh->a_ready[s], PAIR ? 2 * kXfThreads : kXfThreads);
     }
     for (int s = 0; s < 2; ++s) {
       ptx::mbar_init(&sh->tmem_full[s], 1);
-      ptx::mbar_init(&sh->tmem_empty[s], kEpiThreads);
+      ptx::mbar_init(&sh->tmem_empty[s], PAIR ? 2 * kEpiThreads : kEpiThreads);
     }
     for (int s = 0; s < p.nsb && s < kMaxBStages; ++s) {
       ptx::mbar_init(&sh->b_full[s], 1);
@@ -773,8 +793,8 @@
     ptx::fence_barrier_init();
   }
   if (warp == 1) {
-    ptx::tmem_alloc(&sh->tmem_base, (uint32_t)p.tmem_cols);
-    ptx::tmem_relinquish();
+    ptx::tmem_alloc<CG>(&sh->tmem_base, (uint32_t)p.tmem_cols);
+    ptx::tmem_relinquish<CG>();
   }
   float* stat_part = reinterpret_cast<float*>(sh + 1);
   double* stat_acc = reinterpret_cast<double*>(stat_part + 2 * 2 * 8 * p.n_cta);
@@ -783,9 +803,11 @@
     for (int i = threadIdx.x - kEpiFirst; i < 2 * 2 * 8 * p.n_cta; i += kEpiThreads) stat_part[i] = 0.f;
   }
   ptx::tc_fence_before();
-  __syncthreads();
+  if constexpr (PAIR) ptx::cluster_sync();
+  else __syncthreads();
   ptx::tc_fence_after();
   const uint32_t tmem_base = sh->tmem_base;
+  const uint32_t rank = PAIR ? ptx::cluster_ctarank() : 0u;
   constexpr int planes_per_chunk = KJ * 2;
   uint64_t* const a_rdy = p.in_norm ? sh->a_ready : sh->a_full;
   if (warp < 4) {
@@ -795,8 +817,8 @@
     if (lane == 0) {
       uint32_t it = 0;
       Ring ra((uint32_t)p.nsa);
-      for (int tile = blockIdx.x; tile < p.n_tiles; tile += gridDim.x) {
-        const TileCoord t = decode_tile(p, tile);
+      for (int tile = blockIdx.x; tile < tiles_run<PAIR>(p); tile += gridDim.x) {
+        const TileCoord t = decode_tile(p, PAIR && tile >= p.n_tiles ? p.n_tiles - 1 : tile);
         for (int kc = 0; kc < p.k_chunks + p.skip_chunks; ++kc, ++it, ra.next()) {
           const int s = (int)ra.s;
           ptx::mbar_wait(&sh->a_empty[s], ra.ph ^ 1u);
@@ -804,7 +826,12 @@
             ptx::mbar_arrive(&sh->a_full[s]);
             continue;
           }
-          if (kc < p.k_chunks) {
+          if (PAIR && !p.in_norm) {
+            if (rank == 0) ptx::mbar_arrive_expect_tx(&sh->a_full[s], 2u * (uint32_t)(planes_per_chunk * p.plane_bytes));
+            ptx::tma_load_4d_pair(a_smem + (size_t)s * p.a_stage_bytes, &tmap_x, ptx::mapa_shared(&sh->a_full[s], 0),
+                                  (t.w0 - p.pad + p.x_shift) * 8, t.h0 - p.pad + p.x_shift, t.d0 - p.pad + p.x_shift,
+                                  t.b * p.x_planes + p.x_plane0 + kc * planes_per_chunk);
+          } else if (kc < p.k_chunks) {
             ptx::mbar_arrive_expect_tx(&sh->a_full[s], (uint32_t)(planes_per_chunk * p.plane_bytes));
             ptx::tma_load_4d(a_smem + (size_t)s * p.a_stage_bytes, &tmap_x, &sh->a_full[s], (t.w0 - p.pad + p.x_shift) * 8,
                              t.h0 - p.pad + p.x_shift, t.d0 - p.pad + p.x_shift,
@@ -816,6 +843,25 @@
           }
         }
       }
+      if constexpr (PAIR)
+        for (int i = 0; i < p.nsa; ++i, ra.next()) ptx::mbar_wait(&sh->a_empty[ra.s], ra.ph ^ 1u);
+    }
+  } else if (PAIR && (warp == 2 || warp == 3)) {
+    if (warp == 2 && lane == 0) {
+      const int tps = p.taps_per_stage, n_taps = p.n_taps, k_chunks = p.k_chunks;
+      const uint32_t b_stage_bytes = (uint32_t)p.b_stage_bytes;
+      const int row_group0 = (int)rank * (p.n_cta / 16);
+      Ring rb((uint32_t)p.nsb);
+      for (int tile = blockIdx.x; tile < tiles_run<PAIR>(p); tile += gridDim.x)
+        for (int kc = 0; kc < k_chunks; ++kc)
+          for (int tap0 = 0; tap0 < n_taps; tap0 += tps, rb.next()) {
+            const uint32_t s = rb.s;
+            ptx::mbar_wait(&sh->b_empty[s], rb.ph ^ 1u);
+            if (rank == 0) ptx::mbar_arrive_expect_tx(&sh->b_full[s], 2u * b_stage_bytes);
+            ptx::tma_load_4d_pair(b_smem + (size_t)s * b_stage_bytes, &tmap_x2, ptx::mapa_shared(&sh->b_full[s], 0), 0, row_group0,
+                                  kc * planes_per_chunk, tap0);
+          }
+      for (int i = 0; i < p.nsb; ++i, rb.next()) ptx::mbar_wait(&sh->b_empty[rb.s], rb.ph ^ 1u);
     }
   } else if (warp == 2 || warp == 3) {
     const uint32_t pj = (uint32_t)(warp - 2);
@@ -980,39 +1026,46 @@
         }
       }
       }
+    } else if constexpr (PAIR) {
+      if (rank == 0) {
+        if (!p.pad) issue_generic_tiles<MT, KJ, 0, 1, false, kKind, true>(p, sh, a_rdy, a_base16, b_base16, tmem_u, leader);
+        else if (p.taps_per_stage == 3) issue_generic_tiles<MT, KJ, 1, 3, false, kKind, true>(p, sh, a_rdy, a_base16, b_base16, tmem_u, leader);
+        else issue_generic_tiles<MT, KJ, 1, 1, false, kKind, true>(p, sh, a_rdy, a_base16, b_base16, tmem_u, leader);
+      }
     } else {
       const bool res = p.b_resident != 0;
       if (!p.pad) {
-        if (res) issue_generic_tiles<MT, KJ, 0, 1, true, kKind>(p, sh, a_rdy, a_base16, b_base16, tmem_u, leader);
-        else issue_generic_tiles<MT, KJ, 0, 1, false, kKind>(p, sh, a_rdy, a_base16, b_base16, tmem_u, leader);
+        if (res) issue_generic_tiles<MT, KJ, 0, 1, true, kKind, false>(p, sh, a_rdy, a_base16, b_base16, tmem_u, leader);
+        else issue_generic_tiles<MT, KJ, 0, 1, false, kKind, false>(p, sh, a_rdy, a_base16, b_base16, tmem_u, leader);
       } else if (p.taps_per_stage == 3) {
-        if (res) issue_generic_tiles<MT, KJ, 1, 3, true, kKind>(p, sh, a_rdy, a_base16, b_base16, tmem_u, leader);
-        else issue_generic_tiles<MT, KJ, 1, 3, false, kKind>(p, sh, a_rdy, a_base16, b_base16, tmem_u, leader);
+        if (res) issue_generic_tiles<MT, KJ, 1, 3, true, kKind, false>(p, sh, a_rdy, a_base16, b_base16, tmem_u, leader);
+        else issue_generic_tiles<MT, KJ, 1, 3, false, kKind, false>(p, sh, a_rdy, a_base16, b_base16, tmem_u, leader);
       } else {
-        if (res) issue_generic_tiles<MT, KJ, 1, 1, true, kKind>(p, sh, a_rdy, a_base16, b_base16, tmem_u, leader);
-        else issue_generic_tiles<MT, KJ, 1, 1, false, kKind>(p, sh, a_rdy, a_base16, b_base16, tmem_u, leader);
+        if (res) issue_generic_tiles<MT, KJ, 1, 1, true, kKind, false>(p, sh, a_rdy, a_base16, b_base16, tmem_u, leader);
+        else issue_generic_tiles<MT, KJ, 1, 1, false, kKind, false>(p, sh, a_rdy, a_base16, b_base16, tmem_u, leader);
       }
     }
   }
   } else if (warp >= 12) {
     ptx::setmaxnreg_dec<kRegsXf>();
     if constexpr (!TF32)
-      if (p.in_norm) transform_tiles<MT, KJ>(p, sh, a_smem, reinterpret_cast<float*>(smem + p.xf_coef_off));
+      if (p.in_norm) transform_tiles<MT, KJ, PAIR>(p, sh, a_smem, reinterpret_cast<float*>(smem + p.xf_coef_off));
   } else {
     ptx::setmaxnreg_inc<kRegsEpi>();
     constexpr int P = TF32 ? kEpiF32Planar : 0;
-    if (p.out_fp32) epilogue_tiles<MT, kEpiFp32>(p, sh, smem, stat_part, stat_acc, tmem_base);
-    else if (p.residual && p.stats) epilogue_tiles<MT, P | kEpiRes | kEpiStats>(p, sh, smem, stat_part, stat_acc, tmem_base);
-    else if (p.residual) epilogue_tiles<MT, P | kEpiRes>(p, sh, smem, stat_part, stat_acc, tmem_base);
-    else if (p.stats) epilogue_tiles<MT, P | kEpiStats>(p, sh, smem, stat_part, stat_acc, tmem_base);
-    else epilogue_tiles<MT, P>(p, sh, smem, stat_part, stat_acc, tmem_base);
+    if (p.out_fp32) epilogue_tiles<MT, kEpiFp32, PAIR>(p, sh, smem, stat_part, stat_acc, tmem_base);
+    else if (p.residual && p.stats) epilogue_tiles<MT, P | kEpiRes | kEpiStats, PAIR>(p, sh, smem, stat_part, stat_acc, tmem_base);
+    else if (p.residual) epilogue_tiles<MT, P | kEpiRes, PAIR>(p, sh, smem, stat_part, stat_acc, tmem_base);
+    else if (p.stats) epilogue_tiles<MT, P | kEpiStats, PAIR>(p, sh, smem, stat_part, stat_acc, tmem_base);
+    else epilogue_tiles<MT, P, PAIR>(p, sh, smem, stat_part, stat_acc, tmem_base);
   }
 
   ptx::tc_fence_before();
-  __syncthreads();
+  if constexpr (PAIR) ptx::cluster_sync();
+  else __syncthreads();
   if (warp == 1) {
     ptx::tc_fence_after();
-    ptx::tmem_dealloc(tmem_base, (uint32_t)p.tmem_cols);
+    ptx::tmem_dealloc<CG>(tmem_base, (uint32_t)p.tmem_cols);
   }
 }
 
@@ -1024,6 +1077,7 @@
   int no_resident;
   int no_fold;
   int no_march;
+  int pair;
 };
 #ifdef VDM_BRINGUP
 static ConvOverrides g_overrides = {};
@@ -1049,6 +1103,7 @@
   int xf_coef_off;
   size_t smem_bytes;
   int m_units, m_nseg, m_seglen;
+  int pair;
   int debug_flags;
 };
 
@@ -1056,8 +1111,8 @@
   return (d.tap_offset[t][0] + 1) * 9 + (d.tap_offset[t][1] + 1) * 3 + d.tap_offset[t][2] + 1;
 }
 
-static int plan_conv(const VdmConvDesc& d, bool has_residual, bool has_skip, bool has_xf, int skip_c_in, int sms, bool tf32,
-                     ConvPlan& pl) {
+static int plan_conv(const VdmConvDesc& d, bool has_residual, bool has_skip, bool has_xf, int skip_c_in, int sms, int clusters,
+                     bool tf32, ConvPlan& pl) {
   const ConvOverrides& ov = g_overrides;
   pl = ConvPlan{};
   pl.debug_flags = ov.debug_flags;
@@ -1105,9 +1160,10 @@
   const bool resident_fold = pl.schedule == ConvSchedule::kFoldResident || pl.schedule == ConvSchedule::kMarch;
 
   const int tiles_w = ceil_div(d.width, kTileW), tiles_h = ceil_div(d.height, kTileH);
-  int n_split = 1, mt = fold_mt;
+  int n_split = 1, mt = fold_mt, pair = 0;
   if (!fold) {
     double best = -1.0;
+    const bool force_pair = ov.pair == 2 && d.n_taps > 1 && !tf32 && clusters > 0;
     for (int ns = 1; ns <= 8; ns *= 2) {
       if (d.c_out_pad % (ns * 16) != 0) break;
       const int ncta = d.c_out_pad / ns;
@@ -1115,27 +1171,32 @@
       int mt_max = 256 / ncta;
       if (mt_max > 4) mt_max = 4;
       if (mt_max > d.depth) mt_max = d.depth;
-      for (int m = 1; m <= mt_max; ++m) {
-        const long long tiles = (long long)tiles_w * tiles_h * ceil_div(d.depth, m) * d.batch * ns;
-        const long long waves = (tiles + sms - 1) / sms;
-        const double active = (double)(tiles < sms ? tiles : sms);
-        const double fetch_cyc = 32.0 + ncta / 4.0;
-        const double mma_cyc = (double)d.n_taps * (d.c_in / 16) * m * (ncta / 2.0 > fetch_cyc ? ncta / 2.0 : fetch_cyc);
-        const double bytes = (double)(m + 2 * pad) * (kTileH + 2 * pad) * (kTileW + 2 * pad) * d.c_in * 2.0 +
-                             (double)d.n_taps * d.c_in * ncta * 2.0;
-        double bw = 5500.0 / active;
-        if (bw > 64.0) bw = 64.0;
-        const double cyc = (mma_cyc > bytes / bw ? mma_cyc : bytes / bw) + 2000.0;
-        const double total = (double)waves * cyc;
-        if (best < 0.0 || total < best * 0.999) {
-          best = total;
-          n_split = ns;
-          mt = m;
-        }
-      }
-    }
-  }
-  if (ov.force_nsplit > 0) n_split = ov.force_nsplit;
+      const bool pair_ok = ns == 1 && d.n_taps > 1 && !tf32 && clusters > 0 && ov.pair != 1;
+      for (int m = 1; m <= mt_max; ++m)
+        for (int pr = pair_ok ? 1 : 0; pr >= 0; --pr) {
+          if (force_pair && !pr) continue;
+          const long long tiles = (long long)tiles_w * tiles_h * ceil_div(d.depth, m) * d.batch * ns;
+          const long long units = pr ? (tiles + 1) / 2 : tiles, slots = pr ? clusters : sms;
+          const long long waves = (units + slots - 1) / slots;
+          const double active = (double)(pr + 1) * (double)(units < slots ? units : slots);
+          const double fetch_cyc = 32.0 + ncta / (pr ? 8.0 : 4.0);
+          const double mma_cyc = (double)d.n_taps * (d.c_in / 16) * m * (ncta / 2.0 > fetch_cyc ? ncta / 2.0 : fetch_cyc);
+          const double bytes = (double)(m + 2 * pad) * (kTileH + 2 * pad) * (kTileW + 2 * pad) * d.c_in * 2.0 +
+                               (double)d.n_taps * d.c_in * ncta * (pr ? 1.0 : 2.0);
+          double bw = 5500.0 / active;
+          if (bw > 64.0) bw = 64.0;
+          const double cyc = (mma_cyc > bytes / bw ? mma_cyc : bytes / bw) + 2000.0;
+          const double total = (double)waves * cyc;
+          if (best < 0.0 || total < best * 0.999) {
+            best = total;
+            n_split = ns;
+            mt = m;
+            pair = pr;
+          }
+        }
+    }
+  }
+  if (ov.force_nsplit > 0 && ov.force_nsplit != n_split) { n_split = ov.force_nsplit; pair = 0; }
   VDM_CHECK_ARG(d.c_out_pad % (n_split * 16) == 0, "vdm_conv3d: n_split=%d does not divide c_out_pad=%d", n_split,
                 d.c_out_pad);
   const int n_cta = d.c_out_pad / n_split;
@@ -1148,7 +1209,7 @@
               "(3x3x3, c_out_pad 16 or 32, weights + skip weights fit shared memory); c_in=%d c_out=%d", d.c_in, d.c_out);
     return VDM_E_UNSUPPORTED;
   }
-  pl.pad = pad; pl.mt = mt; pl.n_split = n_split; pl.n_cta = n_cta; pl.n_tiles = (int)n_tiles;
+  pl.pad = pad; pl.mt = mt; pl.n_split = n_split; pl.n_cta = n_cta; pl.n_tiles = (int)n_tiles; pl.pair = pair;
   pl.taps_per_stage = (d.n_taps % 3 == 0) ? 3 : 1;
 
   if (pl.schedule == ConvSchedule::kMarch) {
@@ -1203,17 +1264,18 @@
     VDM_CHECK_ARG(2 * pl.a_stage_bytes + pl.b_stage_bytes + skip_w_bytes <= smem_budget,
                   "vdm_conv3d: folded layer does not fit shared memory");
   } else {
+    const int n_b = pair ? n_cta / 2 : n_cta;
     for (int c : {64, 32, 16}) {
       if ((ov.force_kc > 0 && c != ov.force_kc) || d.c_in % c != 0) continue;
       const int a_stage = ((c / 8) * plane_bytes + 127) & ~127;
-      const int b_stage = pl.taps_per_stage * c * n_cta * 2;
+      const int b_stage = pl.taps_per_stage * c * n_b * 2;
       const int room = smem_budget - 2 * a_stage;
       if (room < 2 * b_stage) continue;
       const long long all_b = (long long)d.n_taps * d.c_in * n_cta * 2;
       pl.kc = c;
       pl.a_stage_bytes = a_stage;
       pl.b_stage_bytes = b_stage;
-      pl.b_resident = (n_split == 1 && all_b <= room && ov.no_resident == 0) ? 1 : 0;
+      pl.b_resident = (!pair && n_split == 1 && all_b <= room && ov.no_resident == 0) ? 1 : 0;
       pl.nsb = pl.b_resident ? (int)((all_b + b_stage - 1) / b_stage) : (room / b_stage > kMaxBStages ? kMaxBStages : room / b_stage);
       break;
     }
@@ -1233,7 +1295,12 @@
   }
   pl.xf_coef_off = (used + (int)sizeof(ConvShared) + stat_part_bytes + 16 + pl.res_depth * res_slot + 15) & ~15;
   pl.smem_bytes = (size_t)pl.xf_coef_off + xf_bytes + 1024;
-  pl.grid = pl.n_tiles < sms ? pl.n_tiles : sms;
+  if (pair) {
+    const int pairs = (pl.n_tiles + 1) / 2;
+    pl.grid = 2 * (pairs < clusters ? pairs : clusters);
+  } else {
+    pl.grid = pl.n_tiles < sms ? pl.n_tiles : sms;
+  }
   return VDM_OK;
 }
 
@@ -1264,6 +1331,19 @@
     set_error("vdm_conv3d_tf32: no kernel instance for MT=%d KC=%d", pl.mt, pl.kc / 2);
     return VDM_E_UNSUPPORTED;
   }
+  if (pl.pair) {
+#define VDM_TILE_PAIR(MTv, KJv)                                                                                \
+    if (pl.mt == MTv && pl.kc == 16 * KJv)                                                                     \
+      return launch_kernel_pair<conv3d_planar_kernel<MTv, KJv, 0, false, true>>(pl.grid, kConvThreads, pl.smem_bytes, stream, \
+                                                                                 tmx, tmx2, p);
+    VDM_TILE_PAIR(1, 1) VDM_TILE_PAIR(1, 2) VDM_TILE_PAIR(1, 4)
+    VDM_TILE_PAIR(2, 1) VDM_TILE_PAIR(2, 2) VDM_TILE_PAIR(2, 4)
+    VDM_TILE_PAIR(3, 1) VDM_TILE_PAIR(3, 2) VDM_TILE_PAIR(3, 4)
+    VDM_TILE_PAIR(4, 1) VDM_TILE_PAIR(4, 2) VDM_TILE_PAIR(4, 4)
+#undef VDM_TILE_PAIR
+    set_error("vdm_conv3d: no CTA-pair kernel instance for MT=%d KC=%d", pl.mt, pl.kc);
+    return VDM_E_UNSUPPORTED;
+  }
 #define VDM_TILE(MTv, KJv, NFv)                                                                                \
   if (pl.mt == MTv && pl.kc == 16 * KJv && nf == NFv)                                                          \
     return launch_kernel<conv3d_planar_kernel<MTv, KJv, NFv>>(pl.grid, kConvThreads, pl.smem_bytes, stream, tmx, tmx2, p);
@@ -1294,10 +1374,37 @@
     case 5: g_overrides.debug_flags = value; return VDM_OK;
     case 6: g_overrides.no_fold = value; return VDM_OK;
     case 7: g_overrides.no_march = value; return VDM_OK;
+    case 8: g_overrides.pair = value; return VDM_OK;
     default: set_error("vdm_debug_set: unknown key %d", key); return VDM_E_BADARG;
   }
 }
 #endif
+
+static int pair_clusters() {
+  static int n = []() {
+    auto kernel = conv3d_planar_kernel<2, 2, 0, false, true>;
+    if (cudaFuncSetAttribute(kernel, cudaFuncAttributeMaxDynamicSharedMemorySize, 227 * 1024) != cudaSuccess) {
+      cudaGetLastError();
+      return 0;
+    }
+    cudaLaunchConfig_t cfg = {};
+    cfg.gridDim = dim3(2, 1, 1);
+    cfg.blockDim = dim3(kConvThreads, 1, 1);
+    cfg.dynamicSmemBytes = 227 * 1024;
+    cudaLaunchAttribute attr;
+    attr.id = cudaLaunchAttributeClusterDimension;
+    attr.val.clusterDim.x = 2; attr.val.clusterDim.y = 1; attr.val.clusterDim.z = 1;
+    cfg.attrs = &attr;
+    cfg.numAttrs = 1;
+    int c = 0;
+    if (cudaOccupancyMaxActiveClusters(&c, kernel, &cfg) != cudaSuccess) {
+      cudaGetLastError();
+      return 0;
+    }
+    return c;
+  }();
+  return n;
+}
 
 static int conv3d_run(const VdmConvDesc& d, const void* x, const void* w, void* y, const VdmConvEpilogue* epi, bool tf32,
                       cudaStream_t stream) {
@@ -1332,7 +1439,7 @@
   }
 
   ConvPlan pl;
-  const int rc = plan_conv(d, has_residual, has_skip, has_xf, has_skip ? epi->skip_c_in : 0, num_sms(), tf32, pl);
+  const int rc = plan_conv(d, has_residual, has_skip, has_xf, has_skip ? epi->skip_c_in : 0, num_sms(), pair_clusters(), tf32, pl);
   if (rc != VDM_OK) return rc;
   const int x2_planes = !has_skip ? 0 : epi->skip_planes > 0 ? epi->skip_planes : epi->skip_c_in / 8;
   VDM_CHECK_ARG(!has_skip || (epi->skip_plane0 >= 0 && epi->skip_plane0 + epi->skip_c_in / 8 <= x2_planes),
@@ -1407,6 +1514,19 @@
                         0, {(uint32_t)p.Wh, (uint32_t)p.Hh, box_d, planes}, "vdm_conv3d", march ? "x, marching" : "x");
   if (e != VDM_OK) return e;
   tmx2 = tmx;
+  if (pl.pair) {
+    const cuuint64_t gdim[4] = {64, (cuuint64_t)d.c_out_pad / 8, (cuuint64_t)d.c_in / 8, (cuuint64_t)d.n_taps};
+    const cuuint64_t gstr[3] = {128, (cuuint64_t)d.c_out_pad * 16, (cuuint64_t)d.c_in / 8 * d.c_out_pad * 16};
+    const cuuint32_t bdim[4] = {64, (cuuint32_t)pl.n_cta / 16, (cuuint32_t)pl.kc / 8, (cuuint32_t)pl.taps_per_stage};
+    const cuuint32_t estr[4] = {1, 1, 1, 1};
+    const CUresult r = encode_fn()(&tmx2, CU_TENSOR_MAP_DATA_TYPE_BFLOAT16, 4, const_cast<void*>(w), gdim, gstr, bdim, estr,
+                                   CU_TENSOR_MAP_INTERLEAVE_NONE, CU_TENSOR_MAP_SWIZZLE_NONE, CU_TENSOR_MAP_L2_PROMOTION_L2_256B,
+                                   CU_TENSOR_MAP_FLOAT_OOB_FILL_NONE);
+    if (r != CUDA_SUCCESS) {
+      set_error("vdm_conv3d: cuTensorMapEncodeTiled(w, pair) failed with %d", (int)r);
+      return VDM_E_DRIVER;
+    }
+  }
   if (has_skip) {
     e = encode_planar(&tmx2, epi->skip_x, d.width, d.height, d.depth, (uint64_t)d.batch * x2_planes, 0,
                       {(uint32_t)kTileW, (uint32_t)kTileH, march ? 1u : (uint32_t)pl.mt, planes}, "vdm_conv3d",
diff --git a/vdm4cdm_b200/csrc/ptx.cuh b/vdm4cdm_b200/csrc/ptx.cuh
--- a/vdm4cdm_b200/csrc/ptx.cuh
+++ b/vdm4cdm_b200/csrc/ptx.cuh
@@ -26,41 +26,83 @@
 __device__ __forceinline__ void mbar_arrive(uint64_t* bar) {
   asm volatile("mbarrier.arrive.shared::cta.b64 _, [%0];" ::"r"(smem_u32(bar)) : "memory");
 }
+template <bool CLUSTER = false>
 __device__ __forceinline__ bool mbar_try_wait(uint64_t* bar, uint32_t parity) {
   uint32_t ok;
-  asm volatile(
-      "{\n\t"
-      ".reg .pred p;\n\t"
-      "mbarrier.try_wait.parity.shared::cta.b64 p, [%1], %2;\n\t"
-      "selp.u32 %0, 1, 0, p;\n\t"
-      "}"
-      : "=r"(ok)
-      : "r"(smem_u32(bar)), "r"(parity)
-      : "memory");
+  if constexpr (CLUSTER)
+    asm volatile(
+        "{\n\t"
+        ".reg .pred p;\n\t"
+        "mbarrier.try_wait.parity.acquire.cluster.shared::cta.b64 p, [%1], %2;\n\t"
+        "selp.u32 %0, 1, 0, p;\n\t"
+        "}"
+        : "=r"(ok)
+        : "r"(smem_u32(bar)), "r"(parity)
+        : "memory");
+  else
+    asm volatile(
+        "{\n\t"
+        ".reg .pred p;\n\t"
+        "mbarrier.try_wait.parity.shared::cta.b64 p, [%1], %2;\n\t"
+        "selp.u32 %0, 1, 0, p;\n\t"
+        "}"
+        : "=r"(ok)
+        : "r"(smem_u32(bar)), "r"(parity)
+        : "memory");
   return ok != 0;
 }
+template <bool CLUSTER = false>
 __device__ __forceinline__ bool mbar_try_wait_hint(uint64_t* bar, uint32_t parity, uint32_t hint_ns) {
   uint32_t ok;
-  asm volatile(
-      "{\n\t"
-      ".reg .pred p;\n\t"
-      "mbarrier.try_wait.parity.shared::cta.b64 p, [%1], %2, %3;\n\t"
-      "selp.u32 %0, 1, 0, p;\n\t"
-      "}"
-      : "=r"(ok)
-      : "r"(smem_u32(bar)), "r"(parity), "r"(hint_ns)
-      : "memory");
+  if constexpr (CLUSTER)
+    asm volatile(
+        "{\n\t"
+        ".reg .pred p;\n\t"
+        "mbarrier.try_wait.parity.acquire.cluster.shared::cta.b64 p, [%1], %2, %3;\n\t"
+        "selp.u32 %0, 1, 0, p;\n\t"
+        "}"
+        : "=r"(ok)
+        : "r"(smem_u32(bar)), "r"(parity), "r"(hint_ns)
+        : "memory");
+  else
+    asm volatile(
+        "{\n\t"
+        ".reg .pred p;\n\t"
+        "mbarrier.try_wait.parity.shared::cta.b64 p, [%1], %2, %3;\n\t"
+        "selp.u32 %0, 1, 0, p;\n\t"
+        "}"
+        : "=r"(ok)
+        : "r"(smem_u32(bar)), "r"(parity), "r"(hint_ns)
+        : "memory");
   return ok != 0;
 }
+template <bool CLUSTER = false>
 __device__ __forceinline__ void mbar_wait(uint64_t* bar, uint32_t parity) {
-  if (mbar_try_wait(bar, parity)) return;
+  if (mbar_try_wait<CLUSTER>(bar, parity)) return;
   uint32_t spins = 0;
-  while (!mbar_try_wait_hint(bar, parity, 2000u)) {
+  while (!mbar_try_wait_hint<CLUSTER>(bar, parity, 2000u)) {
     if (++spins > (1u << 21)) {
       printf("vdm4cdm_b200: mbarrier wait timed out (block %d thread %d)\n", (int)blockIdx.x, (int)threadIdx.x);
       __trap();
     }
   }
+}
+
+__device__ __forceinline__ uint32_t cluster_ctarank() {
+  uint32_t r;
+  asm volatile("mov.u32 %0, %%cluster_ctarank;" : "=r"(r));
+  return r;
+}
+__device__ __forceinline__ uint32_t mapa_shared(const void* p, uint32_t rank) {
+  uint32_t a;
+  asm volatile("mapa.shared::cluster.u32 %0, %1, %2;" : "=r"(a) : "r"(smem_u32(p)), "r"(rank));
+  return a;
+}
+__device__ __forceinline__ void mbar_arrive_remote(uint32_t cluster_addr) {
+  asm volatile("mbarrier.arrive.release.cluster.shared::cluster.b64 _, [%0];" ::"r"(cluster_addr) : "memory");
+}
+__device__ __forceinline__ void cluster_sync() {
+  asm volatile("barrier.cluster.arrive.release.aligned;\n\tbarrier.cluster.wait.acquire.aligned;" ::: "memory");
 }
 
 __device__ __forceinline__ bool elect_one() {
@@ -126,6 +168,15 @@
       : "memory");
 }
 
+__device__ __forceinline__ void tma_load_4d_pair(void* dst, const CUtensorMap* m, uint32_t bar_cluster, int c0, int c1, int c2,
+                                                 int c3) {
+  asm volatile(
+      "cp.async.bulk.tensor.4d.cta_group::2.shared::cluster.global.mbarrier::complete_tx::bytes [%0], [%1, {%3, %4, %5, %6}], "
+      "[%2];" ::"r"(smem_u32(dst)),
+      "l"(reinterpret_cast<uint64_t>(m)), "r"(bar_cluster), "r"(c0), "r"(c1), "r"(c2), "r"(c3)
+      : "memory");
+}
+
 __device__ __forceinline__ void bulk_load(void* dst, const void* src, uint32_t bytes, uint64_t* bar) {
   asm volatile("cp.async.bulk.shared::cluster.global.mbarrier::complete_tx::bytes [%0], [%1], %2, [%3];" ::"r"(
                    smem_u32(dst)),
@@ -133,39 +184,54 @@
                : "memory");
 }
 
+template <int CG = 1>
 __device__ __forceinline__ void tmem_alloc(uint32_t* dst_smem, uint32_t ncols) {
-  asm volatile("tcgen05.alloc.cta_group::1.sync.aligned.shared::cta.b32 [%0], %1;" ::"r"(smem_u32(dst_smem)),
-               "r"(ncols)
-               : "memory");
-}
+  if constexpr (CG == 2)
+    asm volatile("tcgen05.alloc.cta_group::2.sync.aligned.shared::cta.b32 [%0], %1;" ::"r"(smem_u32(dst_smem)), "r"(ncols)
+                 : "memory");
+  else
+    asm volatile("tcgen05.alloc.cta_group::1.sync.aligned.shared::cta.b32 [%0], %1;" ::"r"(smem_u32(dst_smem)),
+                 "r"(ncols)
+                 : "memory");
+}
+template <int CG = 1>
 __device__ __forceinline__ void tmem_relinquish() {
-  asm volatile("tcgen05.relinquish_alloc_permit.cta_group::1.sync.aligned;" ::: "memory");
-}
+  if constexpr (CG == 2) asm volatile("tcgen05.relinquish_alloc_permit.cta_group::2.sync.aligned;" ::: "memory");
+  else asm volatile("tcgen05.relinquish_alloc_permit.cta_group::1.sync.aligned;" ::: "memory");
+}
+template <int CG = 1>
 __device__ __forceinline__ void tmem_dealloc(uint32_t taddr, uint32_t ncols) {
-  asm volatile("tcgen05.dealloc.cta_group::1.sync.aligned.b32 %0, %1;" ::"r"(taddr), "r"(ncols) : "memory");
+  if constexpr (CG == 2)
+    asm volatile("tcgen05.dealloc.cta_group::2.sync.aligned.b32 %0, %1;" ::"r"(taddr), "r"(ncols) : "memory");
+  else
+    asm volatile("tcgen05.dealloc.cta_group::1.sync.aligned.b32 %0, %1;" ::"r"(taddr), "r"(ncols) : "memory");
 }
 __device__ __forceinline__ void tc_fence_before() { asm volatile("tcgen05.fence::before_thread_sync;" ::: "memory"); }
 __device__ __forceinline__ void tc_fence_after() { asm volatile("tcgen05.fence::after_thread_sync;" ::: "memory"); }
 
 enum class MmaKind { kF16, kTF32 };
-#define VDM_UMMA_KIND_ASM(K, BODY) \
-  if constexpr (K == MmaKind::kTF32) asm volatile(BODY("tf32")); else asm volatile(BODY("f16"))
-
-#define VDM_UMMA_BODY(KIND)                                                                    \
+#define VDM_UMMA_KIND_ASM(K, CG, BODY)                                                       \
+  if constexpr (CG == 2) {                                                                   \
+    if constexpr (K == MmaKind::kTF32) asm volatile(BODY("2", "tf32")); else asm volatile(BODY("2", "f16")); \
+  } else {                                                                                   \
+    if constexpr (K == MmaKind::kTF32) asm volatile(BODY("1", "tf32")); else asm volatile(BODY("1", "f16")); \
+  }
+
+#define VDM_UMMA_BODY(CG, KIND)                                                                  \
       "{\n\t"                                                                                  \
       ".reg .pred p;\n\t"                                                                      \
       "setp.ne.b32 p, %4, 0;\n\t"                                                              \
-      "tcgen05.mma.cta_group::1.kind::" KIND " [%0], %1, %2, %3, p;\n\t"                       \
+      "tcgen05.mma.cta_group::" CG ".kind::" KIND " [%0], %1, %2, %3, p;\n\t"                   \
       "}" ::"r"(d_tmem),                                                                       \
       "l"(a_desc), "l"(b_desc), "r"(idesc), "r"(accumulate)                                    \
       : "memory"
-template <MmaKind K = MmaKind::kF16>
+template <MmaKind K = MmaKind::kF16, int CG = 1>
 __device__ __forceinline__ void umma_bf16(uint32_t d_tmem, uint64_t a_desc, uint64_t b_desc, uint32_t idesc,
                                           uint32_t accumulate) {
-  VDM_UMMA_KIND_ASM(K, VDM_UMMA_BODY);
+  VDM_UMMA_KIND_ASM(K, CG, VDM_UMMA_BODY);
 }
 #undef VDM_UMMA_BODY
-#define VDM_UMMA_OFF_BODY(KIND)                                                                \
+#define VDM_UMMA_OFF_BODY(CG, KIND)                                                              \
       "{\n\t"                                                                                  \
       ".reg .pred p;\n\t"                                                                      \
       ".reg .b32 alo, blo, dd;\n\t"                                                            \
@@ -176,18 +242,18 @@
       "mov.b64 da, {alo, %3};\n\t"                                                             \
       "mov.b64 db, {blo, %6};\n\t"                                                             \
       "setp.ne.b32 p, %8, 0;\n\t"                                                              \
-      "tcgen05.mma.cta_group::1.kind::" KIND " [dd], da, db, %7, p;\n\t"                       \
+      "tcgen05.mma.cta_group::" CG ".kind::" KIND " [dd], da, db, %7, p;\n\t"                   \
       "}" ::"r"(d_tmem),                                                                       \
       "r"(a_lo), "r"(a_off), "r"(a_hi32), "r"(b_lo), "r"(b_off), "r"(b_hi32), "r"(idesc), "r"(accumulate), "r"(d_off) \
       : "memory"
-template <MmaKind K = MmaKind::kF16>
+template <MmaKind K = MmaKind::kF16, int CG = 1>
 __device__ __forceinline__ void umma_bf16_off(uint32_t d_tmem, uint32_t d_off, uint32_t a_lo, uint32_t a_off, uint32_t a_hi32,
                                               uint32_t b_lo, uint32_t b_off, uint32_t b_hi32, uint32_t idesc,
                                               uint32_t accumulate) {
-  VDM_UMMA_KIND_ASM(K, VDM_UMMA_OFF_BODY);
+  VDM_UMMA_KIND_ASM(K, CG, VDM_UMMA_OFF_BODY);
 }
 #undef VDM_UMMA_OFF_BODY
-#define VDM_UMMA_OFF64_BODY(KIND)                                                              \
+#define VDM_UMMA_OFF64_BODY(CG, KIND)                                                            \
       "{\n\t"                                                                                  \
       ".reg .pred p;\n\t"                                                                      \
       ".reg .b32 dd;\n\t"                                                                      \
@@ -196,19 +262,25 @@
       "add.u64 db, %3, %4;\n\t"                                                                \
       "add.u32 dd, %0, %7;\n\t"                                                                \
       "setp.ne.b32 p, %6, 0;\n\t"                                                              \
-      "tcgen05.mma.cta_group::1.kind::" KIND " [dd], da, db, %5, p;\n\t"                       \
+      "tcgen05.mma.cta_group::" CG ".kind::" KIND " [dd], da, db, %5, p;\n\t"                   \
       "}" ::"r"(d_tmem),                                                                       \
       "l"(a_desc), "l"((uint64_t)a_off), "l"(b_desc), "l"((uint64_t)b_off), "r"(idesc), "r"(accumulate), "r"(d_off) \
       : "memory"
-template <MmaKind K = MmaKind::kF16>
+template <MmaKind K = MmaKind::kF16, int CG = 1>
 __device__ __forceinline__ void umma_bf16_off64(uint32_t d_tmem, uint32_t d_off, uint64_t a_desc, uint32_t a_off, uint64_t b_desc,
                                                 uint32_t b_off, uint32_t idesc, uint32_t accumulate) {
-  VDM_UMMA_KIND_ASM(K, VDM_UMMA_OFF64_BODY);
+  VDM_UMMA_KIND_ASM(K, CG, VDM_UMMA_OFF64_BODY);
 }
 #undef VDM_UMMA_OFF64_BODY
 #undef VDM_UMMA_KIND_ASM
 __device__ __forceinline__ void umma_commit(uint64_t* bar) {
   asm volatile("tcgen05.commit.cta_group::1.mbarrier::arrive::one.shared::cluster.b64 [%0];" ::"r"(smem_u32(bar))
+               : "memory");
+}
+__device__ __forceinline__ void umma_commit_pair(uint64_t* bar, uint16_t cta_mask) {
+  asm volatile("tcgen05.commit.cta_group::2.mbarrier::arrive::one.shared::cluster.multicast::cluster.b64 [%0], %1;" ::"r"(
+                   smem_u32(bar)),
+               "h"(cta_mask)
                : "memory");
 }
 __device__ __forceinline__ void tmem_ld16(uint32_t taddr, uint32_t (&r)[16]) {
diff --git a/vdm4cdm_b200/csrc/tma_host.cuh b/vdm4cdm_b200/csrc/tma_host.cuh
--- a/vdm4cdm_b200/csrc/tma_host.cuh
+++ b/vdm4cdm_b200/csrc/tma_host.cuh
@@ -61,4 +61,26 @@
   return VDM_OK;
 }
 
+template <auto Kernel, typename... Args>
+int launch_kernel_pair(int grid, int threads, size_t smem_bytes, cudaStream_t stream, const Args&... args) {
+  static bool configured = false;
+  if (!configured) {
+    VDM_CHECK_CUDA(cudaFuncSetAttribute(Kernel, cudaFuncAttributeMaxDynamicSharedMemorySize, 227 * 1024));
+    configured = true;
+  }
+  cudaLaunchConfig_t cfg = {};
+  cfg.gridDim = dim3((unsigned)grid, 1, 1);
+  cfg.blockDim = dim3((unsigned)threads, 1, 1);
+  cfg.dynamicSmemBytes = smem_bytes;
+  cfg.stream = stream;
+  cudaLaunchAttribute attr;
+  attr.id = cudaLaunchAttributeClusterDimension;
+  attr.val.clusterDim.x = 2; attr.val.clusterDim.y = 1; attr.val.clusterDim.z = 1;
+  cfg.attrs = &attr;
+  cfg.numAttrs = 1;
+  VDM_CHECK_CUDA(cudaLaunchKernelEx(&cfg, Kernel, args...));
+  VDM_CHECK_LAUNCH();
+  return VDM_OK;
 }
+
+}
```

New measurement: 1.609 billion (median of 6 runs). +2.4%, better.
